# stateless-consensus/phant

Measured on AMD Instinct MI355X. Metric: mpt_proofs_verified_per_sec_depth8, higher is better.
Workload: dtype u64; 1 GPU; config3: 100000 synthetic depth-8 account proofs per GPU against one state root (7 x 532 B full branches + 112 B leaf, 3868 B and 29 Keccak-f per proof, 1% corrupted/exclusion, no cross-proof dedup); every launch sequence in flight verifies its own witness (seeds 2..3: distinct data per slot), 30 back-to-back passes per timed step; parallelism=key-sharded x1, verify_mode=flat, streams=2

## Files before the change

### include/phant_gpu_diag.h

```cpp
#ifndef PHANT_GPU_DIAG_H
#define PHANT_GPU_DIAG_H

#include "phant_gpu.h"

#ifdef __cplusplus
extern "C" {
#endif

PHANT_API int32_t phant_timing(phant_ctx *ctx, int32_t enable);
PHANT_API int32_t phant_last_kernel_ms(phant_ctx *ctx, float *ms);

PHANT_API int32_t phant_verify_stats(phant_ctx *ctx, uint32_t hashed[8]);
PHANT_API int32_t phant_verify_path_stats(phant_ctx *ctx, uint32_t out[2]);
PHANT_API int32_t phant_verify_tier_stats(phant_ctx *ctx, uint32_t out[5]);
PHANT_API int32_t phant_verify_form(phant_ctx *ctx, uint32_t *form);
#define PHANT_VERIFY_KERNEL_STAGES 5
PHANT_API int32_t phant_verify_kernel_ms(phant_ctx *ctx, float ms[PHANT_VERIFY_KERNEL_STAGES]);
PHANT_API int32_t phant_verify_bound_experiment(phant_ctx *ctx, const uint8_t *d_roots, uint32_t n_roots,
                                                const uint32_t *d_root_idx, const uint8_t *d_keys, uint32_t key_len,
                                                const uint8_t *d_nodes, uint64_t nodes_len, const uint64_t *d_node_off,
                                                uint32_t total_nodes, const uint32_t *d_proof_first_node, uint32_t n,
                                                uint8_t *d_status, uint32_t reps, float out_ms[3]);
PHANT_API int32_t phant_keccak_rate(phant_ctx *ctx, uint32_t waves_per_simd, uint32_t perms, double *perms_per_s);

#define PHANT_TRIE_STATS 16
PHANT_API int32_t phant_trie_stats(phant_ctx *ctx, uint32_t out[PHANT_TRIE_STATS]);

PHANT_API int32_t phant_nodeset_tune(phant_ctx *ctx, int32_t form, uint32_t order, uint32_t hash_lds_bytes,
                                     uint32_t resident_wgs);

#define PHANT_NODESET_STATS 14
PHANT_API int32_t phant_nodeset_stats(phant_ctx *ctx, uint32_t out[PHANT_NODESET_STATS]);

#define PHANT_DIAG_SECP_OPS 9
PHANT_API int32_t phant_diag_secp_op(phant_ctx *ctx, uint32_t op, const uint8_t *a, const uint8_t *b, uint32_t n, uint8_t *out);

PHANT_API int32_t phant_diag_scan_u32(phant_ctx *ctx, uint32_t *counters, uint32_t n);
PHANT_API int32_t phant_diag_sort_pairs(phant_ctx *ctx, const uint64_t *keys, const uint32_t *vals, uint32_t n, uint32_t bits,
                                        uint64_t *keys_out, uint32_t *vals_out);
PHANT_API int32_t phant_diag_order_digests(phant_ctx *ctx, const uint8_t *digests, const uint32_t *seg_of, uint32_t n, uint32_t n_seg,
                                           uint32_t prefix_bits, uint32_t *order_out, uint32_t *flag_out);

enum {
    PHANT_DIAG_VERIFY_SERIAL = 1,
    PHANT_DIAG_VERIFY_HASH_LDS_KB,
    PHANT_DIAG_VERIFY_NO_COOP,
    PHANT_DIAG_VERIFY_NO_WAVE,
    PHANT_DIAG_VERIFY_COOP_MAX,
    PHANT_DIAG_STREAM_WGS,
    PHANT_DIAG_STREAM_MB,
    PHANT_DIAG_TRIE_NO_SIDE,
    PHANT_DIAG_TRIE_SIDE_MIN_KEYS,
    PHANT_DIAG_TRIE_AHEAD_MAX_KEYS,
    PHANT_DIAG_TRIE_SIDE_LDS,
    PHANT_DIAG_TRIE_FALLBACK_GRID,
    PHANT_DIAG_TRIE_SLOT_BLOCKS,
    PHANT_DIAG_TRIE_NO_COOP,
    PHANT_DIAG_TRIE_COOP_MAX,
    PHANT_DIAG_TRIE_NO_WAVE,
    PHANT_DIAG_TRIE_JOIN_IN_STREAM,
    PHANT_DIAG_SORT_NO_FALLBACK,
    PHANT_DIAG_SORT_PREFIX_BITS,
    PHANT_DIAG_SORT_REPAIR_BITS,
    PHANT_DIAG_NODESET_WAVE_MAX,
    PHANT_DIAG_TRIE_SMALL_MAX_KEYS,
    PHANT_DIAG_CODE_HASH_FORM,
    PHANT_DIAG_POSTSTATE_RAW_SLOT_KEYS,
    PHANT_DIAG_ADVANCE_ESTIMATE_BYTES,
    PHANT_DIAG_VERIFY_LIST_WGS,
    PHANT_DIAG_RANGES_NO_LEAF_PASS,
    PHANT_DIAG_RANGES_ITEMS_PER_RANGE
};
PHANT_API int32_t phant_diag_set(phant_ctx *ctx, uint32_t knob, int64_t value);

#ifdef __cplusplus
}
#endif
#endif
```

### phant_amd/_lib.py

```python
from __future__ import annotations

import ctypes as C
import os

import torch

_HERE = os.path.dirname(os.path.abspath(__file__))
LIB_PATH = os.path.join(_HERE, "libphant_gpu.so")

OK = 0
E_INVALID_ARG = -1
E_OOM = -2
E_DEVICE = -3
E_NO_DEVICE = -4
E_UNSORTED = -5
E_UNSUPPORTED = -6

PROOF_INVALID_EMPTY = 0
PROOF_PRESENT = 1
PROOF_ABSENT = 2
PROOF_BAD_HASH = 16
PROOF_BAD_RLP = 17
PROOF_BAD_NODE = 18
PROOF_EXTRA_NODES = 19
PROOF_MISSING_NODE = 20
PROOF_BAD_INPUT = 21
PROOF_MISMATCH = 22
PROOF_BAD_VALUE = 23
PROOF_MISSING_SIBLING = 24
RANGE_VALID = 1
RANGE_EMPTY_VALUE = 32
RANGE_VALUE_TOO_LONG = 33
RANGE_BAD_ORDER = 34
RANGE_BELOW_ORIGIN = 35
RANGE_ROOT_MISMATCH = 36
RANGE_NO_LEAF = 0xFFFFFFFF
POST_KEEP, POST_SET, POST_DELETE = 0, 1, 2
PROVE_MAY_REMOVE = 1
ADVANCE_KEEP_OLD = 1
CODE_NONE = 0xFFFFFFFF
SIG_OK, SIG_BAD_RANGE, SIG_HIGH_S, SIG_BAD_RECID, SIG_NOT_ON_CURVE, SIG_INFINITY, SIG_BAD_TX, SIG_BAD_V = range(8)
RECOVER_LOW_S = 1

_vp, _u32, _u64, _i32 = C.c_void_p, C.c_uint32, C.c_uint64, C.c_int32
SYMBOLS = {
    "phant_version": (C.c_char_p, []),
    "phant_device_count": (_i32, []),
    "phant_ctx_create": (_i32, [_vp, C.POINTER(_vp)]),
    "phant_ctx_destroy": (None, [_vp]),
    "phant_last_error": (C.c_char_p, [_vp]),
    "phant_set_stream": (_i32, [_vp, _vp]),
    "phant_stream_sync": (_i32, [_vp]),
    "phant_keccak256": (_i32, [_vp, _vp, _u64, _vp]),
    "phant_keccak256_with_prefix": (_i32, [_vp, _vp, _u64, _vp, _u64, _vp]),
    "phant_keccak256_batch": (_i32, [_vp, _vp, _vp, _u32, _vp]),
    "phant_keccak256_batch_dev": (_i32, [_vp, _vp, _vp, _u32, _vp]),
    "phant_keccak256_fixed_dev": (_i32, [_vp, _vp, _u32, _u64, _u32, _vp]),
    "phant_logs_bloom": (_i32, [_vp, _vp, _vp, _vp, _u32, _u32, _vp]),
    "phant_logs_bloom_dev": (_i32, [_vp, _vp, _vp, _vp, _u32, _u32, _vp]),
    "phant_sender_addresses": (_i32, [_vp, _vp, _u64, _u32, _vp]),
    "phant_sender_addresses_dev": (_i32, [_vp, _vp, _u64, _u32, _vp]),
    "phant_block_receipts": (_i32, [_vp, _vp, _vp]),
    "phant_block_receipts_dev": (_i32, [_vp, _vp, _vp]),
    "phant_header_chain": (_i32, [_vp, _vp, _vp]),
    "phant_header_chain_dev": (_i32, [_vp, _vp, _vp]),
    "phant_headers_decode_rlp": (_i32, [_vp, _vp, _u32, _u32, _vp, _vp]),
    "phant_ecrecover_batch": (_i32, [_vp, _vp, _vp, _vp, _vp, _u32, _u32, _vp, _vp, _vp]),
    "phant_ecrecover_batch_dev": (_i32, [_vp, _vp, _vp, _vp, _vp, _u32, _u32, _vp, _vp, _vp]),
    "phant_tx_senders": (_i32, [_vp, _vp, _vp, _u32, _u64, _vp, _vp]),
    "phant_block_transactions": (_i32, [_vp, _vp, _vp]),
    "phant_block_transactions_dev": (_i32, [_vp, _vp, _vp]),
    "phant_block_transactions_ex": (_i32, [_vp, _vp, _vp]),
    "phant_block_transactions_ex_dev": (_i32, [_vp, _vp, _vp]),
    "phant_block_bodies": (_i32, [_vp, _vp, _vp]),
    "phant_block_bodies_dev": (_i32, [_vp, _vp, _vp]),
    "phant_bodies_decode_rlp": (_i32, [_vp, _vp, _u32, _u32, _vp, _vp]),
    "phant_block_txs_prestate": (_i32, [_vp, _vp, _vp]),
    "phant_block_txs_prestate_dev": (_i32, [_vp, _vp, _vp]),
    "phant_block_settle": (_i32, [_vp, _vp, _vp]),
    "phant_block_settle_dev": (_i32, [_vp, _vp, _vp]),
    "phant_mpt_verify_ranges": (_i32, [_vp, _vp, _vp]),
    "phant_mpt_verify_ranges_dev": (_i32, [_vp, _vp, _vp]),
    "phant_block_access_lists": (_i32, [_vp, _vp, _vp]),
    "phant_block_access_lists_dev": (_i32, [_vp, _vp, _vp]),
    "phant_diag_secp_op": (_i32, [_vp, _u32, _vp, _vp, _u32, _vp]),
    "phant_diag_scan_u32": (_i32, [_vp, _vp, _u32]),
    "phant_diag_sort_pairs": (_i32, [_vp, _vp, _vp, _u32, _u32, _vp, _vp]),
    "phant_diag_order_digests": (_i32, [_vp, _vp, _vp, _u32, _u32, _u32, _vp, _vp]),
    "phant_mpt_verify_batch": (_i32, [_vp, _vp, _u32, _vp, _vp, _u32, _vp, _u64, _vp, _vp, _u32, _vp, _vp, _vp]),
    "phant_mpt_verify_batch_dev": (_i32, [_vp, _vp, _u32, _vp, _vp, _u32, _vp, _u64, _vp, _u32, _vp, _u32, _vp,
                                          _vp, _vp]),
    "phant_mpt_verify_verdict_dev": (_i32, [_vp, _vp, _u32, _vp, _vp, _u32, _vp, _u64, _vp, _u32, _vp, _u32, _vp,
                                            _vp, _vp, _vp]),
    "phant_mpt_verdict_dev": (_i32, [_vp, _vp, _vp, _u32, _u32, _vp]),
    "phant_mpt_verify_nodeset": (_i32, [_vp, _vp, _u32, _vp, _vp, _u32, _vp, _u64, _vp, _u32, _u32, _vp, _vp, _vp]),
    "phant_mpt_verify_nodeset_dev": (_i32, [_vp, _vp, _u32, _vp, _vp, _u32, _vp, _u64, _vp, _u32, _u32, _vp, _vp, _vp]),
    "phant_mpt_verify_nodeset_verdict_dev": (_i32, [_vp, _vp, _u32, _vp, _vp, _u32, _vp, _u64, _vp, _u32, _u32, _vp, _vp, _vp,
                                                    _vp]),
    "phant_mpt_verify_nodeset_submit": (_i32, [_vp, _u32, _vp, _u32, _vp, _vp, _u32, _vp, _u64, _vp, _u32, _u32, _vp, _vp,
                                               _vp]),
    "phant_host_alloc": (_i32, [_vp, C.c_size_t, C.POINTER(_vp)]),
    "phant_host_free": (_i32, [_vp, _vp]),
    "phant_mpt_verify_submit": (_i32, [_vp, _u32, _vp, _u32, _vp, _vp, _u32, _vp, _u64, _vp, _vp, _u32, _vp, _vp, _vp]),
    "phant_wait": (_i32, [_vp, _u32]),
    "phant_witness_parse_json": (_i32, [C.c_char_p, _u64, C.POINTER(_vp), C.c_char_p, _u32]),
    "phant_witness_parse_json_mt": (_i32, [C.c_char_p, _u64, _u32, C.POINTER(_vp), C.c_char_p, _u32]),
    "phant_witness_index_json": (_i32, [C.c_char_p, _u64, _u32, C.POINTER(_vp), C.c_char_p, _u32]),
    "phant_witness_free": (None, [_vp]),
    "phant_witness_get": (_i32, [_vp, _vp]),
    "phant_witness_verify": (_i32, [_vp, _vp, _vp, _vp, C.POINTER(_u32)]),
    "phant_witness_to_json": (_i32, [_vp, _vp, _u64, C.POINTER(_u64)]),
    "phant_exec_witness_parse_json": (_i32, [C.c_char_p, _u64, C.POINTER(_vp), C.c_char_p, _u32]),
    "phant_exec_witness_free": (None, [_vp]),
    "phant_exec_witness_get": (_i32, [_vp, _vp]),
    "phant_exec_witness_prestate": (_i32, [_vp, _vp, _vp, _vp]),
    "phant_exec_witness_poststate": (_i32, [_vp, _vp, _vp, _vp]),
    "phant_exec_witness_advance": (_i32, [_vp, _vp, _vp, _vp, _u32, C.POINTER(_vp)]),
    "phant_mpt_root": (_i32, [_vp, _vp, _vp, _vp, _vp, _u32, _vp]),
    "phant_mpt_root_nodes": (_i32, [_vp, _vp, _vp, _vp, _vp, _u32, _vp, _u32, _vp, _vp, _u32, _vp]),
    "phant_mpt_prove_nodeset": (_i32, [_vp, _vp, _vp, _vp, _vp, _u32, _vp, _u32, _vp, _vp, _vp, _vp, _u32, _vp]),
    "phant_mpt_prove_nodeset_dev": (_i32, [_vp, _vp, _vp, _u64, _vp, _vp, _u64, _u32, _vp, _u32, _vp, _vp, _u64, _vp, _vp, _u32, _vp]),
    "phant_mpt_prove_batch": (_i32, [_vp, _vp, _vp, _vp, _vp, _u32, _vp, _u32, _vp, _vp, _vp, _u32, _vp]),
    "phant_mpt_prove_batch_dev": (_i32, [_vp, _vp, _vp, _u64, _vp, _vp, _u64, _u32, _vp, _u32, _vp, _vp, _u64, _vp, _u32, _vp]),
    "phant_mpt_strip_first_nibble": (_i32, [_vp, _u32, _vp, _u32, C.POINTER(_u32), C.POINTER(_u32)]),
    "phant_index_root_rlp": (_i32, [_vp, _vp, _vp, _u32, _vp]),
    "phant_block_roots": (_i32, [_vp, _vp, _vp, _vp, _u32, _vp, _vp, _vp, _vp, _u32, _u32, _vp]),
    "phant_index_root_be32": (_i32, [_vp, _vp, _vp, _u32, _vp]),
    "phant_state_root": (_i32, [_vp, _vp, _vp, _vp, _vp, _vp, _vp, _vp, _vp, _u32, _vp]),
    "phant_state_witness": (_i32, [_vp, _vp, _vp, _vp, _vp, _vp, _vp, _vp, _vp, _u32, _vp, _vp, _vp, _u32, C.POINTER(_vp), _vp]),
    "phant_state_proofs": (_i32, [_vp, _vp, _vp, _vp, _vp, _vp, _vp, _vp, _vp, _u32, _vp, _vp, _u32, C.POINTER(_vp), _vp]),
    "phant_state_trie_leaves": (_i32, [_vp, _vp, _vp, _vp, _vp, _vp, _vp, _vp, _vp, _u32, _vp, _vp, _u64, _vp]),
    "phant_state_root_dev": (_i32, [_vp, _vp, _vp, _vp, _vp, _vp, _u64, _vp, _vp, _vp, _u32, _u32, _vp]),
    "phant_state_subtrie_nodes": (_i32, [_vp, _vp, _vp, _vp, _vp, _vp, _vp, _vp, _vp, _u32, _vp, _vp, _u32, _vp]),
    "phant_timing": (_i32, [_vp, _i32]),
    "phant_last_kernel_ms": (_i32, [_vp, C.POINTER(C.c_float)]),
    "phant_keccak_rate": (_i32, [_vp, _u32, _u32, C.POINTER(C.c_double)]),
    "phant_nodeset_tune": (_i32, [_vp, _i32, _u32, _u32, _u32]),
    "phant_diag_set": (_i32, [_vp, _u32, C.c_int64]),
    "phant_verify_kernel_ms": (_i32, [_vp, C.POINTER(C.c_float * 5)]),
    "phant_verify_form": (_i32, [_vp, C.POINTER(C.c_uint32)]),
    "phant_verify_bound_experiment": (_i32, [_vp, _vp, _u32, _vp, _vp, _u32, _vp, _u64, _vp, _u32, _vp, _u32, _vp, _u32,
                                            C.POINTER(C.c_float * 3)]),
    "phant_verify_stats": (_i32, [_vp, C.POINTER(C.c_uint32 * 8)]),
    "phant_verify_path_stats": (_i32, [_vp, C.POINTER(C.c_uint32 * 2)]),
    "phant_verify_tier_stats": (_i32, [_vp, C.POINTER(C.c_uint32 * 5)]),
    "phant_trie_stats": (_i32, [_vp, C.POINTER(C.c_uint32 * 16)]),
    "phant_nodeset_stats": (_i32, [_vp, C.POINTER(C.c_uint32 * 14)]),
    "phant_mpt_root_dev": (_i32, [_vp, _vp, _vp, _u64, _vp, _vp, _u64, _u32, _vp]),
    "phant_comm_create": (_i32, [_vp, _u32, _u32, C.POINTER(_vp)]),
    "phant_comm_destroy": (None, [_vp]),
    "phant_comm_size": (_u32, [_vp]),
    "phant_comm_ctx": (_vp, [_vp, _u32]),
    "phant_comm_last_error": (C.c_char_p, [_vp]),
    "phant_comm_owner": (_u32, [_vp, _vp, _u32]),
    "phant_mpt_verify_sharded": (_i32, [_vp, _vp, _u32, _vp, _vp, _u32, _vp, _u64, _vp, _vp, _u32, _vp, _vp, _vp, _vp]),
    "phant_mpt_verify_nodeset_sharded": (_i32, [_vp, _vp, _u32, _vp, _vp, _u32, _vp, _u64, _vp, _u32, _vp, _u32, _vp, _vp, _vp,
                                                _vp]),
    "phant_mpt_root_sharded": (_i32, [_vp, _vp, _vp, _vp, _vp, _u32, _vp]),
    "phant_state_root_sharded": (_i32, [_vp, _vp, _vp, _vp, _vp, _vp, _vp, _vp, _vp, _u32, _vp]),
    "phant_comm_allreduce_verdict": (_i32, [_vp, _vp, _u32]),
}


class PhantOpts(C.Structure):
    _fields_ = [("struct_size", C.c_uint32), ("device", C.c_int32), ("stream", C.c_void_p), ("flags", C.c_uint32)]


class PhantReceiptsIn(C.Structure):
    _fields_ = [("struct_size", C.c_uint32), ("n_receipts", C.c_uint32), ("n_logs", C.c_uint32), ("n_topics", C.c_uint32),
                ("data_bytes", C.c_uint64), ("tx_type", C.c_void_p), ("status", C.c_void_p), ("cum_gas", C.c_void_p),
                ("log_first", C.c_void_p), ("address", C.c_void_p), ("topic_first", C.c_void_p), ("data_off", C.c_void_p),
                ("topics", C.c_void_p), ("data", C.c_void_p), ("lists", C.c_void_p), ("list_off", C.c_void_p),
                ("list_n", C.c_void_p), ("list_bytes", C.c_void_p), ("n_lists", C.c_uint32), ("receipts_at", C.c_uint32)]


class PhantReceiptsOut(C.Structure):
    _fields_ = [("struct_size", C.c_uint32), ("encoded_off_cap", C.c_uint32), ("encoded_cap", C.c_uint64),
                ("receipts_root", C.c_void_p), ("logs_bloom", C.c_void_p), ("blooms", C.c_void_p), ("encoded", C.c_void_p),
                ("encoded_off", C.c_void_p), ("roots_out", C.c_void_p), ("encoded_len", C.c_uint64)]


HEADER_ARRAYS = ("parent_hash", "uncle_hash", "fee_recipient", "state_root", "transactions_root", "receipts_root", "logs_bloom", "difficulty",
                 "number", "gas_limit", "gas_used", "timestamp", "extra_data", "extra_off", "prev_randao", "nonce", "base_fee",
                 "withdrawals_root", "blob_gas_used", "excess_blob_gas", "parent_beacon_root", "requests_hash", "n_fields", "seg_first",
                 "expected_hash")
HEADERS_FROM_BLOCKS = 1


class PhantHeadersIn(C.Structure):
    _fields_ = [("struct_size", C.c_uint32), ("n", C.c_uint32), ("n_segs", C.c_uint32), ("reserved", C.c_uint32)] + \
               [(name, C.c_void_p) for name in HEADER_ARRAYS]


class PhantHeadersOut(C.Structure):
    _fields_ = [("struct_size", C.c_uint32), ("first_bad", C.c_uint32), ("enc_cap", C.c_uint64), ("hashes", C.c_void_p),
                ("flags", C.c_void_p), ("enc", C.c_void_p), ("enc_off", C.c_void_p), ("enc_len", C.c_uint64)]


TXS_HAVE_GAS_LIMIT, TXS_NO_RECOVERY = 1, 2
TX_OUTPUTS = (("tx_hash", "u1", 32), ("sig_hash", "u1", 32), ("sender", "u1", 20), ("sig_status", "u1", 1), ("sig", "u1", 65), ("type", "u1", 1),
              ("chain_id", "u8", 1), ("nonce", "u8", 1), ("gas_limit", "u8", 1), ("gas_price", "u1", 32), ("priority_fee", "u1", 32),
              ("value", "u1", 32), ("to", "u1", 20), ("data_off", "u8", 1), ("data_len", "u4", 1), ("al_off", "u8", 1), ("al_len", "u4", 1),
              ("al_addresses", "u4", 1), ("al_keys", "u4", 1), ("intrinsic_gas", "u8", 1), ("effective_gas_price", "u1", 32),
              ("upfront_cost", "u1", 32), ("flags", "u4", 1))
TX_FLAG_NAMES = ("Undecodable", "BadV", "Signature", "ChainId", "PriorityAboveMax", "FeeBelowBase", "GasAboveBlock", "IntrinsicGas", "NonceMax",
                 "InitcodeSize", "CostOverflow", "IsCreate")
TX_ERROR_BITS = 0x7FF


class PhantTxsIn(C.Structure):
    _fields_ = [("struct_size", C.c_uint32), ("n", C.c_uint32), ("flags", C.c_uint32), ("reserved", C.c_uint32), ("txs", C.c_void_p),
                ("tx_off", C.c_void_p), ("tx_bytes", C.c_uint64), ("chain_id", C.c_uint64), ("base_fee", C.c_void_p),
                ("block_gas_limit", C.c_uint64)]


class PhantTxsOut(C.Structure):
    _fields_ = [("struct_size", C.c_uint32), ("first_bad", C.c_uint32)] + [(name, C.c_void_p) for name, _, _ in TX_OUTPUTS]


TXS_FORK_LONDON, TXS_FORK_CANCUN, TXS_FORK_PRAGUE = 0, 1, 2
AUTH_CHAIN_ID, AUTH_NONCE_MAX = 8, 9
TX_EX_OUTPUTS = (("max_fee_per_blob_gas", "u1", 32), ("blob_off", "u8", 1), ("blobs", "u4", 1), ("auth_first", "u4", 1), ("floor_gas", "u8", 1))
TX_AUTH_OUTPUTS = (("auth_chain_id", "u1", 32), ("auth_address", "u1", 20), ("auth_nonce", "u8", 1), ("auth_hash", "u1", 32), ("auth_sig", "u1", 65),
                   ("authority", "u1", 20), ("auth_status", "u1", 1))
TX_FLAG_NAMES_EX = TX_FLAG_NAMES + ("NoTo", "BlobNone", "BlobVersion", "BlobFeeBelowBase", "AuthNone", "FloorGas")
TX_ERROR_BITS_EX = 0x7FF | 0x7F000


def tx_error_bits(fork=None):
    return TX_ERROR_BITS if fork is None else TX_ERROR_BITS_EX


class PhantTxsExIn(C.Structure):
    _fields_ = [("struct_size", C.c_uint32), ("fork", C.c_uint32), ("base", PhantTxsIn), ("blob_base_fee", C.c_void_p), ("auth_cap", C.c_uint32),
                ("reserved", C.c_uint32)]


class PhantTxsExOut(C.Structure):
    _fields_ = [("struct_size", C.c_uint32), ("n_auth", C.c_uint32), ("blob_gas_used", C.c_uint64), ("base", PhantTxsOut)] + \
               [(name, C.c_void_p) for name, _, _ in TX_EX_OUTPUTS + TX_AUTH_OUTPUTS]


BODY_TX, BODY_TXS_ROOT, BODY_WD_ROOT, BODY_BLOB_GAS = 1, 2, 4, 8
BODY_FLAG_NAMES = ("Transaction", "TransactionsRoot", "WithdrawalsRoot", "BlobGasUsed")
BODIES_INPUTS = ("txs", "tx_off", "block_first", "withdrawals", "wd_off", "wd_first", "base_fee", "gas_limit", "blob_base_fee", "transactions_root",
                 "withdrawals_root", "blob_gas_used")
BODIES_OUTPUTS = (("tx_block", "u4", 1, "n"), ("block_first_bad", "u4", 1, "n_blocks"), ("block_blob_gas_used", "u8", 1, "n_blocks"),
                  ("transactions_root", "u1", 32, "n_blocks"), ("withdrawals_root", "u1", 32, "n_blocks"), ("block_flags", "u4", 1, "n_blocks"))


BODIES_NO_HEADER = 1
BODIES_SPLIT_ARRAYS = ("txs", "tx_off", "block_first", "withdrawals", "wd_off", "wd_first")


class PhantBodiesSplit(C.Structure):
    _fields_ = [(name, C.c_uint32) for name in ("struct_size", "reserved", "tx_cap", "wd_cap")] + [("tx_bytes_cap", C.c_uint64), ("wd_bytes_cap", C.c_uint64)] + \
               [(name, C.c_void_p) for name in BODIES_SPLIT_ARRAYS] + [("n", C.c_uint32), ("n_wd", C.c_uint32), ("tx_bytes", C.c_uint64), ("wd_bytes", C.c_uint64)]


class PhantBodiesIn(C.Structure):
    _fields_ = [(name, C.c_uint32) for name in ("struct_size", "fork", "flags", "n_blocks", "n", "n_wd", "auth_cap", "reserved")] + \
               [("chain_id", C.c_uint64), ("txs", C.c_void_p), ("tx_off", C.c_void_p), ("tx_bytes", C.c_uint64), ("block_first", C.c_void_p),
                ("withdrawals", C.c_void_p), ("wd_off", C.c_void_p), ("wd_bytes", C.c_uint64)] + \
               [(name, C.c_void_p) for name in BODIES_INPUTS[5:]]


class PhantBodiesOut(C.Structure):
    _fields_ = [("struct_size", C.c_uint32), ("first_bad_block", C.c_uint32), ("txs", PhantTxsExOut)] + \
               [(name, C.c_void_p) for name, _, _, _ in BODIES_OUTPUTS]


ROW_NONE = 0xFFFFFFFF
TXSTATE_INPUTS = ("sender", "sig_status", "tx_flags", "nonce", "upfront_cost", "to", "auth_first", "authority", "auth_status", "addresses",
                  "account_status", "nonces", "balances", "code_hashes", "code_index", "code_off", "codes")
TXSTATE_OUTPUTS = (("sender_row", "u4", 1, "n"), ("to_row", "u4", 1, "n"), ("expected_nonce", "u8", 1, "n"), ("spent_before", "u1", 32, "n"),
                   ("state_flags", "u4", 1, "n"), ("sends", "u4", 1, "n_accounts"), ("roles", "u1", 1, "n_accounts"), ("probe_row", "u4", 1, "n_probe"))
TXST_FLAG_NAMES = ("SenderUnknown", "ToUnknown", "NonceLow", "NonceHigh", "BalanceShort", "NotEOA", "CodeMissing", None, "Skipped", "Undetermined",
                   "NeedsInflow", "SpentSaturated")
TXST_ERROR_BITS = 0x7F
TXST_SKIPPED, TXST_UNDETERMINED, TXST_NEEDS_INFLOW, TXST_SPENT_SATURATED = 0x100, 0x200, 0x400, 0x800
ROLE_SENDER, ROLE_RECIPIENT, ROLE_AUTHORITY, ROLE_PROBE = 1, 2, 4, 8


class PhantTxstateIn(C.Structure):
    _fields_ = [(name, C.c_uint32) for name in ("struct_size", "fork", "n", "n_auth", "n_accounts", "n_codes", "n_probe", "reserved")] + \
               [(name, C.c_void_p) for name in TXSTATE_INPUTS] + [("code_bytes", C.c_uint64), ("probe", C.c_void_p)]


class PhantTxstateOut(C.Structure):
    _fields_ = [(name, C.c_uint32) for name in ("struct_size", "first_bad", "n_undetermined", "reserved")] + \
               [(name, C.c_void_p) for name, _, _, _ in TXSTATE_OUTPUTS]


# ... 88 lines not shown
```

### phant_amd/context.py

```python
from __future__ import annotations

import ctypes as C

import numpy as np
import torch

from . import _lib as L


def _np_ptr(a: np.ndarray):
    return a.ctypes.data_as(C.c_void_p)


class Context:

    def __init__(self, device: int | None = None, use_torch_stream: bool = True, verify_nodedup: bool = False,
                 dedup_levels: int | None = None):
        lib = L.lib()
        if not torch.cuda.is_available():
            raise L.PhantError(L.E_NO_DEVICE, "no GPU visible (phant_amd has no CPU fallback)")
        if device is None:
            device = torch.cuda.current_device()
        self.device = int(device)
        stream, flags = None, 1
        if use_torch_stream:
            stream, flags = torch.cuda.current_stream(self.device).cuda_stream or None, 0
        if verify_nodedup:
            dedup_levels = 0
        if dedup_levels is not None:
            flags |= ((int(dedup_levels) + 1) << 8) & 0x1F00
        opts = L.PhantOpts(C.sizeof(L.PhantOpts), self.device, stream, flags)
        h = C.c_void_p()
        rc = lib.phant_ctx_create(C.byref(opts), C.byref(h))
        if rc != L.OK:
            raise L.PhantError(rc, "phant_ctx_create failed (needs a gfx950 device)")
        self._h = h
        self._lib = lib

    @classmethod
    def borrowed(cls, handle, device: int) -> "Context":
        self = cls.__new__(cls)
        self.device = int(device)
        self._lib = L.lib()
        self._h = handle
        self._borrowed = True
        return self

    def check(self, rc: int):
        if rc != L.OK:
            raise L.PhantError(rc, self._lib.phant_last_error(self._h).decode())

    def sync(self):
        self.check(self._lib.phant_stream_sync(self._h))

    def timing(self, enable: bool):
        self.check(self._lib.phant_timing(self._h, 1 if enable else 0))

    def last_kernel_ms(self) -> float:
        ms = C.c_float(0)
        self.check(self._lib.phant_last_kernel_ms(self._h, C.byref(ms)))
        return ms.value

    def keccak_rate(self, waves_per_simd: int = 6, perms: int = 100) -> float:
        out = C.c_double(0.0)
        self.check(self._lib.phant_keccak_rate(self._h, waves_per_simd, perms, C.byref(out)))
        return out.value

    VERIFY_STAGES = ("propose", "hash_deep", "dedup", "hash_list", "walk")
    VERIFY_FORMS = {0: "hash_everything", 1: "two_tiers"}
    DIAG = {name: k + 1 for k, name in enumerate((
        "verify_serial", "verify_hash_lds_kb", "verify_no_coop", "verify_no_wave", "verify_coop_max", "stream_wgs", "stream_mb",
        "trie_no_side", "trie_side_min_keys", "trie_ahead_max_keys", "trie_side_lds", "trie_fallback_grid", "trie_slot_blocks",
        "trie_no_coop", "trie_coop_max", "trie_no_wave", "trie_join_in_stream", "sort_no_fallback", "sort_prefix_bits",
        "sort_repair_bits", "nodeset_wave_max", "trie_small_max_keys", "code_hash_form", "poststate_raw_slot_keys",
        "advance_estimate_bytes", "verify_list_wgs", "ranges_no_leaf_pass", "ranges_items_per_range"))}

    def diag_set(self, knob: str, value: int):
        self.check(self._lib.phant_diag_set(self._h, self.DIAG[knob], int(value)))

    def nodeset_tune(self, form: int = 1, order: int = 0, hash_lds: int = 40 * 1024, resident_wgs: int = 0):
        self.check(self._lib.phant_nodeset_tune(self._h, form, order, hash_lds, resident_wgs))

    def verify_kernel_ms(self) -> dict[str, float]:
        out = (C.c_float * 5)()
        self.check(self._lib.phant_verify_kernel_ms(self._h, C.byref(out)))
        return dict(zip(self.VERIFY_STAGES, [float(x) for x in out]))

    def verify_bound_experiment(self, batch, reps: int = 20) -> dict[str, float]:
        import torch
        st = torch.empty(batch.n, dtype=torch.uint8, device=batch.nodes.device)
        out = (C.c_float * 3)()
        self.check(self._lib.phant_verify_bound_experiment(
            self._h, batch.roots.data_ptr(), batch.n_roots, None if batch.root_idx is None else batch.root_idx.data_ptr(),
            batch.keys.data_ptr(), batch.key_len, batch.nodes.data_ptr(), batch.nodes.numel(), batch.node_off.data_ptr(),
            batch.node_off.numel() - 1, batch.proof_first_node.data_ptr(), batch.n, st.data_ptr(), reps, C.byref(out)))
        return {"hash_only_ms": float(out[0]), "stream_only_ms": float(out[1]), "together_ms": float(out[2])}

    def verify_form(self) -> str:
        out = C.c_uint32(0)
        self.check(self._lib.phant_verify_form(self._h, C.byref(out)))
        return self.VERIFY_FORMS.get(int(out.value), "?")

    def verify_stats(self) -> list[int]:
        out = (C.c_uint32 * 8)()
        self.check(self._lib.phant_verify_stats(self._h, C.byref(out)))
        return list(out)

    def verify_tier_stats(self) -> dict[str, int]:
        out = (C.c_uint32 * 5)()
        self.check(self._lib.phant_verify_tier_stats(self._h, C.byref(out)))
        return dict(zip(("dedup_levels", "list_nodes", "list_keccak_f", "deep_nodes", "deep_keccak_f"), [int(x) for x in out]))

    TRIE_PASSES = {0: "none", 1: "small", 2: "general"}

    def trie_stats(self) -> dict:
        out = (C.c_uint32 * 16)()
        self.check(self._lib.phant_trie_stats(self._h, C.byref(out)))
        v = [int(x) for x in out]
        return {"pass": self.TRIE_PASSES.get(v[0], "?"), "leaves_ahead": bool(v[1]), "deep_from": v[2] - (1 << 32) if v[2] >> 31 else v[2],
                "bins": v[3], "max_bin": v[4], "wave": v[5], "half_wave": v[6], "blocks1": v[7], "blocks2": v[8], "blocks4": v[9],
                "misfits": v[10], "leaf_big": bool(v[11]), "n_rep": v[12], "n": v[13], "side_bins": v[14], "scratch_bytes": v[15]}

    def nodeset_stats(self) -> list[int]:
        out = (C.c_uint32 * 14)()
        self.check(self._lib.phant_nodeset_stats(self._h, C.byref(out)))
        return [int(x) for x in out]

    def verify_path_stats(self) -> tuple[int, int]:
        out = (C.c_uint32 * 2)()
        self.check(self._lib.phant_verify_path_stats(self._h, C.byref(out)))
        return int(out[0]), int(out[1])

    def close(self):
        if getattr(self, "_h", None):
            if not getattr(self, "_borrowed", False):
                self._lib.phant_ctx_destroy(self._h)
            self._h = None

    def __del__(self):
        try:
            self.close()
        except Exception:
            pass

    @property
    def handle(self):
        return self._h


_default: dict[int, Context] = {}


def default_context(device: int | None = None) -> Context:
    if device is None:
        device = torch.cuda.current_device() if torch.cuda.is_available() else 0
    ctx = _default.get(device)
    if ctx is None:
        ctx = Context(device)
        _default[device] = ctx
    return ctx
```

### phant_amd/csrc/capi.hip

```cpp
#include <hip/hip_runtime.h>

#include <algorithm>
#include <cstdio>
#include <cstdlib>
#include <cstring>
#include <memory>
#include <new>
#include <random>
#include <string>
#include <vector>

#include "../../include/phant_gpu.h"
#include "../../include/phant_gpu_diag.h"
#include "arena.h"
#include "staging.h"
#include "launch.h"
#include "receipts.h"
#include "headers.h"
#include "transactions.h"
#include "settle.h"
#include "txstate.h"
#include "access_lists.h"
#include "trie_build.h"
#include "witness.h"
// ... 168 lines not shown
    DeviceGuard g(dev);
    if (!own) {
        c->stream = (hipStream_t)stream;
    } else {
        if (hipStreamCreateWithFlags(&c->stream, hipStreamNonBlocking) != hipSuccess) {
            c->stream = nullptr;
            return PHANT_E_DEVICE;
        }
        c->own_stream = true;
    }
    if (hipEventCreate(&c->ev0) != hipSuccess || hipEventCreate(&c->ev1) != hipSuccess) return PHANT_E_DEVICE;
    c->tune.last_shallow = &c->last_shallow;
    c->tune.last_form = &c->last_form;
    holder.c = nullptr;
    *out = c;
    return PHANT_OK;
}

void phant_ctx_destroy(phant_ctx* c) {
    if (!c) return;
    DeviceGuard g(c->device);
    (void)hipStreamSynchronize(c->stream);
    c->ws.release();
    c->dv.release();
    c->ns.dv.release();
    if (c->secp_gtable) (void)hipFree(c->secp_gtable);
    if (c->ev0) (void)hipEventDestroy(c->ev0);
    if (c->ev1) (void)hipEventDestroy(c->ev1);
    for (hipEvent_t e : c->kev)
        if (e) (void)hipEventDestroy(e);
    for (auto& sl : c->slots) {
        if (sl.stream) {
            (void)hipStreamSynchronize(sl.stream);
            (void)hipStreamDestroy(sl.stream);
        }
        sl.io.release();
        sl.dv.release();
        sl.ns.dv.release();
    }
    if (c->side.stream) (void)hipStreamSynchronize(c->side.stream);
    if (c->side.stream2) (void)hipStreamSynchronize(c->side.stream2);
    if (c->side.fork) (void)hipEventDestroy(c->side.fork);
    if (c->side.join) (void)hipEventDestroy(c->side.join);
    if (c->side.join2) (void)hipEventDestroy(c->side.join2);
    if (c->code_side.stream) (void)hipStreamSynchronize(c->code_side.stream);
    if (c->code_side.fork) (void)hipEventDestroy(c->code_side.fork);
    if (c->code_side.join) (void)hipEventDestroy(c->code_side.join);
    if (c->code_side.stream) (void)hipStreamDestroy(c->code_side.stream);
    if (c->side.stream) (void)hipStreamDestroy(c->side.stream);
    if (c->side.stream2) (void)hipStreamDestroy(c->side.stream2);
    if (c->own_stream && c->stream) (void)hipStreamDestroy(c->stream);
    delete c;
}

const char* phant_last_error(const phant_ctx* c) { return c ? c->err.c_str() : "null ctx"; }

int32_t phant_set_stream(phant_ctx* c, void* stream) {
    if (!c) return PHANT_E_INVALID_ARG;
    DeviceGuard g(c->device);
    HIP_TRY(c, hipStreamSynchronize(c->stream));
    if (c->own_stream) {
        (void)hipStreamDestroy(c->stream);
        c->own_stream = false;
    }
    c->stream = (hipStream_t)stream;
    return PHANT_OK;
}

int32_t phant_stream_sync(phant_ctx* c) {
    if (!c) return PHANT_E_INVALID_ARG;
    DeviceGuard g(c->device);
    HIP_TRY(c, hipStreamSynchronize(c->stream));
    return PHANT_OK;
}

int32_t phant_timing(phant_ctx* c, int32_t enable) {
    if (!c) return PHANT_E_INVALID_ARG;
    c->timing = enable != 0;
    c->ev_pending = false;
    return PHANT_OK;
}

int32_t phant_verify_stats(phant_ctx* c, uint32_t hashed[8]) {
    if (!c || !hashed) return PHANT_E_INVALID_ARG;
    for (int i = 0; i < 8; ++i) hashed[i] = 0;
    if (c->last_was_nodeset) {
        if (!c->ns.dv.base) return PHANT_OK;
        DeviceGuard g(c->device);
        HIP_TRY(c, hipStreamSynchronize(c->stream));
        uint32_t hdr[phant::VERIFY_HEADER_WORDS];
        HIP_TRY(c, hipMemcpy(hdr, c->ns.dv.base, sizeof(hdr), hipMemcpyDeviceToHost));
        phant::verify_nodeset_stats_from_header(hdr, c->ns.epoch, hashed, nullptr);
        return PHANT_OK;
    }
    if (!c->dv.base) return PHANT_OK;
    DeviceGuard g(c->device);
    HIP_TRY(c, hipStreamSynchronize(c->stream));
    if (c->side.stream) HIP_TRY(c, hipStreamSynchronize(c->side.stream));
    uint32_t hdr[phant::VERIFY_HEADER_WORDS];
    HIP_TRY(c, hipMemcpy(hdr, c->dv.base, sizeof(hdr), hipMemcpyDeviceToHost));
    phant::verify_stats_from_header(hdr, hashed);
    return PHANT_OK;
}

int32_t phant_nodeset_stats(phant_ctx* c, uint32_t out[PHANT_NODESET_STATS]) {
    if (!c || !out) return PHANT_E_INVALID_ARG;
    for (int i = 0; i < PHANT_NODESET_STATS; ++i) out[i] = 0;
    if (!c->ns.dv.base || c->ns.dirty || c->ns.epoch == 0u || c->ns_last[0] == 0u) return PHANT_OK;
    DeviceGuard g(c->device);
    HIP_TRY(c, hipStreamSynchronize(c->stream));
    uint32_t hdr[phant::VERIFY_HEADER_WORDS];
    HIP_TRY(c, hipMemcpy(hdr, c->ns.dv.base, sizeof(hdr), hipMemcpyDeviceToHost));
    uint32_t hashed[8], overflow = 0;
    phant::verify_nodeset_stats_from_header(hdr, c->ns.epoch, hashed, &overflow);
    phant::verify_nodeset_lists_from_header(hdr, c->ns.epoch, out + 1);
    out[0] = c->ns_last[0];
    out[10] = overflow;
    out[11] = c->ns_last[1];
    out[12] = c->ns_last[2];
    out[13] = c->ns.epoch;
    return PHANT_OK;
}

int32_t phant_verify_tier_stats(phant_ctx* c, uint32_t out[5]) {
    if (!c || !out) return PHANT_E_INVALID_ARG;
    for (int i = 0; i < 5; ++i) out[i] = 0;
    if (!c->dv.base) return PHANT_OK;
    DeviceGuard g(c->device);
    HIP_TRY(c, hipStreamSynchronize(c->stream));
    if (c->side.stream) HIP_TRY(c, hipStreamSynchronize(c->side.stream));
    uint32_t hdr[phant::VERIFY_HEADER_WORDS];
    HIP_TRY(c, hipMemcpy(hdr, c->dv.base, sizeof(hdr), hipMemcpyDeviceToHost));
    out[0] = c->last_shallow;
    phant::verify_tier_stats_from_header(hdr, out + 1);
    return PHANT_OK;
}

int32_t phant_verify_form(phant_ctx* c, uint32_t* form) {
    if (!c || !form) return PHANT_E_INVALID_ARG;
    *form = c->last_form;
    return PHANT_OK;
}

int32_t phant_verify_path_stats(phant_ctx* c, uint32_t out[2]) {
    if (!c || !out) return PHANT_E_INVALID_ARG;
    out[0] = out[1] = 0;
    if (!c->dv.base) return PHANT_OK;
    DeviceGuard g(c->device);
    HIP_TRY(c, hipStreamSynchronize(c->stream));
    if (c->side.stream) HIP_TRY(c, hipStreamSynchronize(c->side.stream));
    uint32_t hdr[phant::VERIFY_HEADER_WORDS];
    HIP_TRY(c, hipMemcpy(hdr, c->dv.base, sizeof(hdr), hipMemcpyDeviceToHost));
    phant::verify_paths_from_header(hdr, out);
    return PHANT_OK;
}

int32_t phant_trie_stats(phant_ctx* c, uint32_t out[PHANT_TRIE_STATS]) {
    if (!c || !out) return PHANT_E_INVALID_ARG;
    const phant::TrieStats& s = c->ws.trie_stats;
    for (int i = 0; i < PHANT_TRIE_STATS; ++i) out[i] = 0;
    out[0] = s.pass;
    out[1] = s.ahead;
    out[2] = (uint32_t)s.deep_from;
    out[3] = s.bins;
    out[4] = s.max_bin;
    for (int k = 0; k < 5; ++k) out[5 + k] = s.by_class[k];
    out[11] = s.leaf_big;
    out[12] = s.n_rep;
    out[13] = s.n;
    out[14] = s.side_bins;
    DeviceGuard g(c->device);
    HIP_TRY(c, hipStreamSynchronize(c->stream));
    if (c->ws.side) HIP_TRY(c, hipStreamSynchronize(c->ws.side));
    constexpr size_t MISFIT_BYTES = 512 * sizeof(uint32_t);
    if (s.has_misfit && c->ws.t1.base && s.misfit_off + MISFIT_BYTES <= c->ws.t1.cap) {
        std::vector<uint32_t> mis(512);
        HIP_TRY(c, hipMemcpy(mis.data(), c->ws.t1.base + s.misfit_off, MISFIT_BYTES, hipMemcpyDeviceToHost));
        uint64_t tot = 0;
        for (const uint32_t m : mis) tot += m;
        out[10] = (uint32_t)std::min<uint64_t>(tot, 0xffffffffull);
    }
    if (s.has_cursor && c->ws.t1.base && s.cursor_off + sizeof(unsigned long long) <= c->ws.t1.cap) {
        unsigned long long used = 0;
        HIP_TRY(c, hipMemcpy(&used, c->ws.t1.base + s.cursor_off, sizeof used, hipMemcpyDeviceToHost));
        out[15] = (uint32_t)std::min<unsigned long long>(used, 0xffffffffull);
    }
    return PHANT_OK;
}

int32_t phant_verify_kernel_ms(phant_ctx* c, float ms[PHANT_VERIFY_KERNEL_STAGES]) {
    if (!c || !ms) return PHANT_E_INVALID_ARG;
    if (!c->tune.kernel_ev) return fail(c, PHANT_E_UNSUPPORTED, "verify_kernel_ms: the tiers are not serialised on this ctx (phant_diag_set: the verify-serial knob)");
    if (!c->kev_valid) return fail(c, PHANT_E_INVALID_ARG, "verify_kernel_ms: the last verify launch on this ctx was not a two-tier one");
    DeviceGuard g(c->device);
    HIP_TRY(c, hipStreamSynchronize(c->stream));
    static_assert(PHANT_VERIFY_KERNEL_STAGES == phant::VERIFY_KERNEL_STAGES, "one stage list");
    for (int i = 0; i < PHANT_VERIFY_KERNEL_STAGES; ++i) {
        ms[i] = 0.f;
        if (hipEventElapsedTime(&ms[i], c->kev[i], c->kev[i + 1]) != hipSuccess) {
            (void)hipGetLastError();
            return fail(c, PHANT_E_INVALID_ARG, "verify_kernel_ms: no two-tier launch on this ctx yet");
        }
    }
    return PHANT_OK;
}

int32_t phant_last_kernel_ms(phant_ctx* c, float* ms) {
    if (!c || !ms) return PHANT_E_INVALID_ARG;
    if (!c->ev_pending) return fail(c, PHANT_E_INVALID_ARG, "no timed call pending");
    DeviceGuard g(c->device);
    HIP_TRY(c, hipEventSynchronize(c->ev1));
    HIP_TRY(c, hipEventElapsedTime(ms, c->ev0, c->ev1));
    return PHANT_OK;
}

int32_t phant_diag_set(phant_ctx* c, uint32_t knob, int64_t value) {
    if (!c) return PHANT_E_INVALID_ARG;
    DeviceGuard g(c->device);
    phant::TrieTune& t = c->ws.tune;
    switch (knob) {
        case PHANT_DIAG_VERIFY_SERIAL:
            if (value && !c->tune.kernel_ev) {
                for (hipEvent_t& e : c->kev)
                    if (!e) HIP_TRY(c, hipEventCreate(&e));
                c->tune.kernel_ev = c->kev;
            }
            c->tune.serial = value != 0;
            c->kev_valid = false;
            return PHANT_OK;
        case PHANT_DIAG_VERIFY_HASH_LDS_KB:
            c->tune.hash_lds = (uint32_t)(value < 0 ? 0 : value > 47 ? 47 : value) * 1024u;
            return PHANT_OK;
        case PHANT_DIAG_VERIFY_NO_COOP: c->tune.no_coop = value != 0; return PHANT_OK;
        case PHANT_DIAG_VERIFY_NO_WAVE: c->tune.no_wave = value != 0; return PHANT_OK;
        case PHANT_DIAG_VERIFY_COOP_MAX: c->tune.coop_max = (uint32_t)(value < 0 ? 0 : value > (1 << 20) ? (1 << 20) : value); return PHANT_OK;
        case PHANT_DIAG_STREAM_WGS: c->tune.diag_stream_wgs = (uint32_t)(value < 0 ? 0 : value > 65536 ? 65536 : value); return PHANT_OK;
        case PHANT_DIAG_STREAM_MB: c->tune.diag_stream_mb = (uint32_t)(value < 0 ? 0 : value > 65536 ? 65536 : value); return PHANT_OK;
        case PHANT_DIAG_TRIE_NO_SIDE: t.no_side = value != 0; return PHANT_OK;
        case PHANT_DIAG_TRIE_SIDE_MIN_KEYS: t.side_min_keys = value; return PHANT_OK;
        case PHANT_DIAG_TRIE_AHEAD_MAX_KEYS: t.ahead_max_keys = value; return PHANT_OK;
        case PHANT_DIAG_TRIE_SIDE_LDS: t.side_lds = value; return PHANT_OK;
        case PHANT_DIAG_TRIE_FALLBACK_GRID: t.fallback_grid = value; return PHANT_OK;
        case PHANT_DIAG_TRIE_SLOT_BLOCKS: t.slot_blocks = (int32_t)value; return PHANT_OK;
        case PHANT_DIAG_TRIE_NO_COOP: t.no_coop = value != 0; return PHANT_OK;
        case PHANT_DIAG_TRIE_COOP_MAX: t.coop_max = value; return PHANT_OK;
        case PHANT_DIAG_TRIE_NO_WAVE: t.no_wave = value != 0; return PHANT_OK;
        case PHANT_DIAG_TRIE_JOIN_IN_STREAM: t.join_in_stream = value != 0; return PHANT_OK;
        case PHANT_DIAG_SORT_NO_FALLBACK: t.sort_no_fallback = value != 0; return PHANT_OK;
        case PHANT_DIAG_SORT_PREFIX_BITS: t.sort_prefix_bits = value; return PHANT_OK;
        case PHANT_DIAG_SORT_REPAIR_BITS: t.sort_repair_bits = value; return PHANT_OK;
        case PHANT_DIAG_NODESET_WAVE_MAX: c->ns_tune.wave_max = (uint32_t)(value < 0 ? 0 : value > (1 << 20) ? (1 << 20) : value); return PHANT_OK;
        case PHANT_DIAG_TRIE_SMALL_MAX_KEYS: t.small_max_keys = value; return PHANT_OK;
        case PHANT_DIAG_CODE_HASH_FORM: c->code_form = value == 1 ? 1u : 0u; return PHANT_OK;
        case PHANT_DIAG_POSTSTATE_RAW_SLOT_KEYS: c->post_raw_slot_keys = value != 0; return PHANT_OK;
        case PHANT_DIAG_ADVANCE_ESTIMATE_BYTES: c->advance_estimate = value > 0 ? (uint64_t)value : 0u; return PHANT_OK;
        case PHANT_DIAG_VERIFY_LIST_WGS: c->tune.list_wgs_cap = (uint32_t)(value < 0 ? 0 : value > (1 << 20) ? (1 << 20) : value); return PHANT_OK;
        case PHANT_DIAG_RANGES_NO_LEAF_PASS: c->ranges_no_leaf_pass = value != 0; return PHANT_OK;
        case PHANT_DIAG_RANGES_ITEMS_PER_RANGE: c->ranges_items_per_range = value < 0 ? -1 : value > 1922 ? 1922 : value; return PHANT_OK;
        default: return fail(c, PHANT_E_INVALID_ARG, "diag_set: no such knob");
    }
}

int32_t phant_nodeset_tune(phant_ctx* c, int32_t ladder, uint32_t order, uint32_t hash_lds_bytes, uint32_t resident_wgs) {
    if (!c || ladder < 0 || ladder > 2 || order > 1u || hash_lds_bytes > 56u * 1024u) return PHANT_E_INVALID_ARG;
    c->ns_tune.form = (uint32_t)ladder;
    c->ns_tune.order = order;
    c->ns_tune.hash_lds = hash_lds_bytes;
    c->ns_tune.resident_wgs = resident_wgs;
    return PHANT_OK;
}

int32_t phant_keccak_rate(phant_ctx* c, uint32_t waves_per_simd, uint32_t perms, double* perms_per_s) {
    if (!c || !perms_per_s || waves_per_simd == 0 || waves_per_simd > 8 || perms == 0) return PHANT_E_INVALID_ARG;
    DeviceGuard g(c->device);
    int cus = 0;
    HIP_TRY(c, hipDeviceGetAttribute(&cus, hipDeviceAttributeMultiprocessorCount, c->device));
    const uint32_t blocks = (uint32_t)cus * waves_per_simd;
    uint32_t* d_out = nullptr;
    const int32_t rc = lay_out(c, c->stream, c->ws.io, [&](auto& io) { d_out = io.template take<uint32_t>((size_t)blocks * 256); });
    if (rc) return rc;
    hipEvent_t e0 = nullptr, e1 = nullptr;
    HIP_TRY(c, hipEventCreate(&e0));
    hipError_t e = hipEventCreate(&e1);
    if (e == hipSuccess) e = phant::launch_keccak_rate(d_out, blocks, perms, c->stream);
    if (e == hipSuccess) e = hipEventRecord(e0, c->stream);
    if (e == hipSuccess) e = phant::launch_keccak_rate(d_out, blocks, perms, c->stream);
    if (e == hipSuccess) e = hipEventRecord(e1, c->stream);
    if (e == hipSuccess) e = hipEventSynchronize(e1);
    float ms = 0.f;
    if (e == hipSuccess) e = hipEventElapsedTime(&ms, e0, e1);
    (void)hipEventDestroy(e0);
    if (e1) (void)hipEventDestroy(e1);
    if (e != hipSuccess) return fail(c, PHANT_E_DEVICE, "keccak_rate", e);
    *perms_per_s = ms > 0.f ? (double)blocks * 256.0 * perms / (ms * 1e-3) : 0.0;
    return PHANT_OK;
}


int32_t phant_keccak256_batch_dev(phant_ctx* c, const uint8_t* d_blob, const uint64_t* d_off,
                                  uint32_t n, uint8_t* d_out) {
    if (!c) return PHANT_E_INVALID_ARG;
    if (n == 0) return PHANT_OK;
    if (!d_off || !d_out || !aligned16(d_out)) return fail(c, PHANT_E_INVALID_ARG, "keccak256_batch_dev: null or unaligned pointer");
    DeviceGuard g(c->device);
    TimedRegion t(c);
    HIP_TRY(c, phant::launch_keccak256_var(d_blob, d_off, n, d_out, c->stream));
    return PHANT_OK;
}

int32_t phant_keccak256_fixed_dev(phant_ctx* c, const uint8_t* d_blob, uint32_t msg_len,
                                  uint64_t stride, uint32_t n, uint8_t* d_out) {
    if (!c) return PHANT_E_INVALID_ARG;
    if (n == 0) return PHANT_OK;
    if (!d_out || !aligned16(d_out) || (!d_blob && msg_len) || (stride < msg_len && n > 1))
        return fail(c, PHANT_E_INVALID_ARG, "keccak256_fixed_dev: bad argument");
    DeviceGuard g(c->device);
    TimedRegion t(c);
    HIP_TRY(c, phant::launch_keccak256_fixed(d_blob, msg_len, stride, n, d_out, c->stream));
    return PHANT_OK;
}

int32_t phant_keccak256_batch(phant_ctx* c, const uint8_t* blob, const uint64_t* off, uint32_t n,
                              uint8_t* out) {
    if (!c) return PHANT_E_INVALID_ARG;
    if (n == 0) return PHANT_OK;
    if (!off || !out) return fail(c, PHANT_E_INVALID_ARG, "keccak256_batch: null pointer");
    for (uint32_t i = 0; i < n; ++i)
        if (off[i + 1] < off[i]) return fail(c, PHANT_E_INVALID_ARG, "keccak256_batch: offsets not monotone");
    const uint64_t lo = off[0], hi = off[n];
    const size_t blob_len = (size_t)(hi - lo);
    if (blob_len && !blob) return fail(c, PHANT_E_INVALID_ARG, "keccak256_batch: null blob");
    DeviceGuard g(c->device);
    uint8_t *d_blob = nullptr, *d_out = nullptr;
    uint64_t* d_off = nullptr;
    const int32_t rc = lay_out(c, c->stream, c->ws.io, [&](auto& io) {
        d_blob = io.template take<uint8_t>(blob_len + 16);
        d_off = io.template take<uint64_t>((size_t)n + 1);
        d_out = io.template take<uint8_t>((size_t)n * 32);
    });
    if (rc) return rc;
    std::vector<uint64_t> rel((size_t)n + 1);
    for (uint32_t i = 0; i <= n; ++i) rel[i] = off[i] - lo;
    if (blob_len) HIP_TRY(c, hipMemcpyAsync(d_blob, blob + lo, blob_len, hipMemcpyHostToDevice, c->stream));
    HIP_TRY(c, hipMemcpyAsync(d_off, rel.data(), rel.size() * 8, hipMemcpyHostToDevice, c->stream));
    HIP_TRY(c, phant::launch_keccak256_var(d_blob, d_off, n, d_out, c->stream));
    HIP_TRY(c, hipMemcpyAsync(out, d_out, (size_t)n * 32, hipMemcpyDeviceToHost, c->stream));
    HIP_TRY(c, hipStreamSynchronize(c->stream));
    return PHANT_OK;
}

int32_t phant_keccak256(phant_ctx* c, const uint8_t* data, uint64_t len, uint8_t out[32]) {
    const uint64_t off[2] = {0, len};
    return phant_impl::phant_keccak256_batch(c, data, off, 1, out);
}

int32_t phant_keccak256_with_prefix(phant_ctx* c, const uint8_t* prefix, uint64_t prefix_len,
                                    const uint8_t* data, uint64_t len, uint8_t out[32]) {
    if (!c) return PHANT_E_INVALID_ARG;
    if ((prefix_len && !prefix) || (len && !data)) return fail(c, PHANT_E_INVALID_ARG, "keccak256_with_prefix: null pointer");
    uint8_t* cat = (uint8_t*)std::malloc((size_t)(prefix_len + len) + 1);
    if (!cat) return fail(c, PHANT_E_OOM, "keccak256_with_prefix: host staging");
    if (prefix_len) std::memcpy(cat, prefix, (size_t)prefix_len);
    if (len) std::memcpy(cat + prefix_len, data, (size_t)len);
    const uint64_t off[2] = {0, prefix_len + len};
    const int32_t rc = phant_impl::phant_keccak256_batch(c, cat, off, 1, out);
    std::free(cat);
    return rc;
}


int32_t phant_logs_bloom_dev(phant_ctx* c, const uint8_t* d_items, const uint64_t* d_item_off,
                             const uint32_t* d_item_receipt, uint32_t n_items, uint32_t n_receipts, uint8_t* d_blooms) {
    if (!c) return PHANT_E_INVALID_ARG;
    if (n_receipts == 0) return PHANT_OK;
    if (!d_blooms || ((uintptr_t)d_blooms & 3u) || (n_items && (!d_item_off || !d_item_receipt)))
        return fail(c, PHANT_E_INVALID_ARG, "logs_bloom_dev: null or unaligned pointer");
    DeviceGuard g(c->device);
    TimedRegion t(c);
    HIP_TRY(c, phant::launch_logs_bloom(d_items, d_item_off, d_item_receipt, n_items, n_receipts, d_blooms, c->stream));
    return PHANT_OK;
}

int32_t phant_logs_bloom(phant_ctx* c, const uint8_t* items, const uint64_t* item_off, const uint32_t* item_receipt,
                         uint32_t n_items, uint32_t n_receipts, uint8_t* blooms) {
    if (!c) return PHANT_E_INVALID_ARG;
    if (n_receipts == 0) return PHANT_OK;
    if (!blooms || (n_items && (!item_off || !item_receipt))) return fail(c, PHANT_E_INVALID_ARG, "logs_bloom: null pointer");
    for (uint32_t i = 0; i < n_items; ++i)
        if (item_off[i + 1] < item_off[i]) return fail(c, PHANT_E_INVALID_ARG, "logs_bloom: offsets not monotone");
    const uint64_t lo = n_items ? item_off[0] : 0, hi = n_items ? item_off[n_items] : 0;
    const size_t blob_len = (size_t)(hi - lo);
    if (blob_len && !items) return fail(c, PHANT_E_INVALID_ARG, "logs_bloom: null items");
    DeviceGuard g(c->device);
    uint8_t *d_items = nullptr, *d_blooms = nullptr;
    uint64_t* d_off = nullptr;
    uint32_t* d_rcpt = nullptr;
    const int32_t rc = lay_out(c, c->stream, c->ws.io, [&](auto& io) {
        d_items = io.template take<uint8_t>(blob_len + 16);
        d_off = io.template take<uint64_t>((size_t)n_items + 1);
        d_rcpt = io.template take<uint32_t>((size_t)n_items + 1);
        d_blooms = io.template take<uint8_t>((size_t)n_receipts * 256);
    });
    if (rc) return rc;
    std::vector<uint64_t> rel((size_t)n_items + 1, 0);
    for (uint32_t i = 0; i <= n_items && n_items; ++i) rel[i] = item_off[i] - lo;
    if (blob_len) HIP_TRY(c, hipMemcpyAsync(d_items, items + lo, blob_len, hipMemcpyHostToDevice, c->stream));
    HIP_TRY(c, hipMemcpyAsync(d_off, rel.data(), rel.size() * 8, hipMemcpyHostToDevice, c->stream));
    if (n_items) HIP_TRY(c, hipMemcpyAsync(d_rcpt, item_receipt, (size_t)n_items * 4, hipMemcpyHostToDevice, c->stream));
    HIP_TRY(c, phant::launch_logs_bloom(d_items, d_off, d_rcpt, n_items, n_receipts, d_blooms, c->stream));
// ... 2200 lines not shown
```

### phant_amd/csrc/capi_guard_capi.inc

```
extern "C" {

const char * phant_version(void) {
    try { return phant_impl::phant_version(); } catch (...) { return nullptr; }
}

int32_t phant_device_count(void) {
    try { return phant_impl::phant_device_count(); }
    catch (const std::bad_alloc&) { return phant_impl::guard_failed(nullptr, PHANT_E_OOM); }
    catch (...) { return phant_impl::guard_failed(nullptr, PHANT_E_DEVICE); }
}

int32_t phant_ctx_create(const phant_opts *opts, phant_ctx **out) {
    try { return phant_impl::phant_ctx_create(opts, out); }
    catch (const std::bad_alloc&) { return phant_impl::guard_failed(nullptr, PHANT_E_OOM); }
    catch (...) { return phant_impl::guard_failed(nullptr, PHANT_E_DEVICE); }
}

void phant_ctx_destroy(phant_ctx *ctx) {
    try { phant_impl::phant_ctx_destroy(ctx); } catch (...) {}
}

const char * phant_last_error(const phant_ctx *ctx) {
    try { return phant_impl::phant_last_error(ctx); } catch (...) { return nullptr; }
}
// ... 330 lines not shown
    catch (...) { return phant_impl::guard_failed(ctx, PHANT_E_DEVICE); }
}

int32_t phant_exec_witness_advance(phant_ctx *ctx, const phant_exec_witness *w, const uint8_t *parent_state_root, phant_poststate *io, uint32_t flags, phant_exec_witness **next) {
    try { return phant_impl::phant_exec_witness_advance(ctx, w, parent_state_root, io, flags, next); }
    catch (const std::bad_alloc&) { return phant_impl::guard_failed(ctx, PHANT_E_OOM); }
    catch (...) { return phant_impl::guard_failed(ctx, PHANT_E_DEVICE); }
}

int32_t phant_mpt_root(phant_ctx *ctx, const uint8_t *keys, const uint32_t *key_off, const uint8_t *vals, const uint64_t *val_off, uint32_t n, uint8_t out[32]) {
    try { return phant_impl::phant_mpt_root(ctx, keys, key_off, vals, val_off, n, out); }
    catch (const std::bad_alloc&) { return phant_impl::guard_failed(ctx, PHANT_E_OOM); }
    catch (...) { return phant_impl::guard_failed(ctx, PHANT_E_DEVICE); }
}

int32_t phant_mpt_root_dev(phant_ctx *ctx, const uint8_t *d_keys, const uint32_t *d_key_off, uint64_t key_bytes, const uint8_t *d_vals, const uint64_t *d_val_off, uint64_t val_bytes, uint32_t n, uint8_t *d_root) {
    try { return phant_impl::phant_mpt_root_dev(ctx, d_keys, d_key_off, key_bytes, d_vals, d_val_off, val_bytes, n, d_root); }
    catch (const std::bad_alloc&) { return phant_impl::guard_failed(ctx, PHANT_E_OOM); }
    catch (...) { return phant_impl::guard_failed(ctx, PHANT_E_DEVICE); }
}

int32_t phant_mpt_prove_nodeset(phant_ctx *ctx, const uint8_t *keys, const uint32_t *key_off, const uint8_t *vals, const uint64_t *val_off, uint32_t n, const uint32_t *seg_first , uint32_t n_tries, const uint8_t *qkeys, const uint32_t *qkey_off , const uint32_t *q_trie , const uint8_t *q_flags , uint32_t n_queries, phant_prove_out *out) {
    try { return phant_impl::phant_mpt_prove_nodeset(ctx, keys, key_off, vals, val_off, n, seg_first, n_tries, qkeys, qkey_off, q_trie, q_flags, n_queries, out); }
    catch (const std::bad_alloc&) { return phant_impl::guard_failed(ctx, PHANT_E_OOM); }
    catch (...) { return phant_impl::guard_failed(ctx, PHANT_E_DEVICE); }
}

int32_t phant_mpt_prove_nodeset_dev(phant_ctx *ctx, const uint8_t *d_keys, const uint32_t *d_key_off, uint64_t key_bytes, const uint8_t *d_vals, const uint64_t *d_val_off, uint64_t val_bytes, uint32_t n, const uint32_t *d_seg_first , uint32_t n_tries, const uint8_t *d_qkeys, const uint32_t *d_qkey_off, uint64_t qkey_bytes, const uint32_t *d_q_trie , const uint8_t *d_q_flags , uint32_t n_queries, phant_prove_out *out) {
    try { return phant_impl::phant_mpt_prove_nodeset_dev(ctx, d_keys, d_key_off, key_bytes, d_vals, d_val_off, val_bytes, n, d_seg_first, n_tries, d_qkeys, d_qkey_off, qkey_bytes, d_q_trie, d_q_flags, n_queries, out); }
    catch (const std::bad_alloc&) { return phant_impl::guard_failed(ctx, PHANT_E_OOM); }
    catch (...) { return phant_impl::guard_failed(ctx, PHANT_E_DEVICE); }
}

int32_t phant_mpt_prove_batch(phant_ctx *ctx, const uint8_t *keys, const uint32_t *key_off, const uint8_t *vals, const uint64_t *val_off, uint32_t n, const uint32_t *seg_first , uint32_t n_tries, const uint8_t *qkeys, const uint32_t *qkey_off , const uint32_t *q_trie , uint32_t n_queries, phant_prove_batch_out *out) {
    try { return phant_impl::phant_mpt_prove_batch(ctx, keys, key_off, vals, val_off, n, seg_first, n_tries, qkeys, qkey_off, q_trie, n_queries, out); }
    catch (const std::bad_alloc&) { return phant_impl::guard_failed(ctx, PHANT_E_OOM); }
    catch (...) { return phant_impl::guard_failed(ctx, PHANT_E_DEVICE); }
}

int32_t phant_mpt_prove_batch_dev(phant_ctx *ctx, const uint8_t *d_keys, const uint32_t *d_key_off, uint64_t key_bytes, const uint8_t *d_vals, const uint64_t *d_val_off, uint64_t val_bytes, uint32_t n, const uint32_t *d_seg_first , uint32_t n_tries, const uint8_t *d_qkeys, const uint32_t *d_qkey_off, uint64_t qkey_bytes, const uint32_t *d_q_trie , uint32_t n_queries, phant_prove_batch_out *out) {
    try { return phant_impl::phant_mpt_prove_batch_dev(ctx, d_keys, d_key_off, key_bytes, d_vals, d_val_off, val_bytes, n, d_seg_first, n_tries, d_qkeys, d_qkey_off, qkey_bytes, d_q_trie, n_queries, out); }
    catch (const std::bad_alloc&) { return phant_impl::guard_failed(ctx, PHANT_E_OOM); }
    catch (...) { return phant_impl::guard_failed(ctx, PHANT_E_DEVICE); }
}

int32_t phant_index_root_rlp(phant_ctx *ctx, const uint8_t *items, const uint64_t *item_off, uint32_t n, uint8_t out[32]) {
    try { return phant_impl::phant_index_root_rlp(ctx, items, item_off, n, out); }
    catch (const std::bad_alloc&) { return phant_impl::guard_failed(ctx, PHANT_E_OOM); }
    catch (...) { return phant_impl::guard_failed(ctx, PHANT_E_DEVICE); }
}

int32_t phant_index_root_be32(phant_ctx *ctx, const uint8_t *items, const uint64_t *item_off, uint32_t n, uint8_t out[32]) {
    try { return phant_impl::phant_index_root_be32(ctx, items, item_off, n, out); }
    catch (const std::bad_alloc&) { return phant_impl::guard_failed(ctx, PHANT_E_OOM); }
    catch (...) { return phant_impl::guard_failed(ctx, PHANT_E_DEVICE); }
}

int32_t phant_block_roots(phant_ctx *ctx, const uint8_t *const *items, const uint64_t *const *item_off, const uint32_t *n, uint32_t n_lists, uint8_t *roots_out, const uint8_t *bloom_items, const uint64_t *bloom_item_off, const uint32_t *bloom_item_receipt, uint32_t n_bloom_items, uint32_t n_receipts, uint8_t *blooms) {
    try { return phant_impl::phant_block_roots(ctx, items, item_off, n, n_lists, roots_out, bloom_items, bloom_item_off, bloom_item_receipt, n_bloom_items, n_receipts, blooms); }
    catch (const std::bad_alloc&) { return phant_impl::guard_failed(ctx, PHANT_E_OOM); }
    catch (...) { return phant_impl::guard_failed(ctx, PHANT_E_DEVICE); }
}

int32_t phant_mpt_verify_ranges(phant_ctx *ctx, const phant_ranges_in *in, phant_ranges_out *out) {
    try { return phant_impl::phant_mpt_verify_ranges(ctx, in, out); }
    catch (const std::bad_alloc&) { return phant_impl::guard_failed(ctx, PHANT_E_OOM); }
    catch (...) { return phant_impl::guard_failed(ctx, PHANT_E_DEVICE); }
}

int32_t phant_mpt_verify_ranges_dev(phant_ctx *ctx, const phant_ranges_in *in, phant_ranges_out *out) {
    try { return phant_impl::phant_mpt_verify_ranges_dev(ctx, in, out); }
    catch (const std::bad_alloc&) { return phant_impl::guard_failed(ctx, PHANT_E_OOM); }
    catch (...) { return phant_impl::guard_failed(ctx, PHANT_E_DEVICE); }
}

int32_t phant_mpt_root_nodes(phant_ctx *ctx, const uint8_t *keys, const uint32_t *key_off, const uint8_t *vals, const uint64_t *val_off, uint32_t n, const uint32_t *seg_first , uint32_t n_tries, uint8_t *roots , uint8_t *node_rlp , uint32_t node_cap, uint32_t *node_len) {
    try { return phant_impl::phant_mpt_root_nodes(ctx, keys, key_off, vals, val_off, n, seg_first, n_tries, roots, node_rlp, node_cap, node_len); }
    catch (const std::bad_alloc&) { return phant_impl::guard_failed(ctx, PHANT_E_OOM); }
    catch (...) { return phant_impl::guard_failed(ctx, PHANT_E_DEVICE); }
}

int32_t phant_mpt_strip_first_nibble(const uint8_t *node, uint32_t len, uint8_t *out, uint32_t cap, uint32_t *out_len, uint32_t *is_ref) {
    try { return phant_impl::phant_mpt_strip_first_nibble(node, len, out, cap, out_len, is_ref); }
    catch (const std::bad_alloc&) { return phant_impl::guard_failed(nullptr, PHANT_E_OOM); }
    catch (...) { return phant_impl::guard_failed(nullptr, PHANT_E_DEVICE); }
}

int32_t phant_state_root(phant_ctx *ctx, const uint8_t *addrs, const uint64_t *nonces, const uint8_t *balances, const uint8_t *code, const uint64_t *code_off, const uint8_t *slot_keys, const uint8_t *slot_vals, const uint32_t *slot_first, uint32_t n, uint8_t out[32]) {
    try { return phant_impl::phant_state_root(ctx, addrs, nonces, balances, code, code_off, slot_keys, slot_vals, slot_first, n, out); }
    catch (const std::bad_alloc&) { return phant_impl::guard_failed(ctx, PHANT_E_OOM); }
    catch (...) { return phant_impl::guard_failed(ctx, PHANT_E_DEVICE); }
}

int32_t phant_state_root_dev(phant_ctx *ctx, const uint8_t *d_addrs, const uint64_t *d_nonces, const uint8_t *d_balances, const uint8_t *d_code, const uint64_t *d_code_off, uint64_t code_bytes, const uint8_t *d_slot_keys, const uint8_t *d_slot_vals, const uint32_t *d_slot_first, uint32_t n_slots, uint32_t n, uint8_t *d_root) {
    try { return phant_impl::phant_state_root_dev(ctx, d_addrs, d_nonces, d_balances, d_code, d_code_off, code_bytes, d_slot_keys, d_slot_vals, d_slot_first, n_slots, n, d_root); }
    catch (const std::bad_alloc&) { return phant_impl::guard_failed(ctx, PHANT_E_OOM); }
    catch (...) { return phant_impl::guard_failed(ctx, PHANT_E_DEVICE); }
}

int32_t phant_state_witness(phant_ctx *ctx, const uint8_t *addrs, const uint64_t *nonces, const uint8_t *balances, const uint8_t *code, const uint64_t *code_off, const uint8_t *slot_keys, const uint8_t *slot_vals, const uint32_t *slot_first, uint32_t n, const uint8_t *wkeys, const uint32_t *wkey_off , const uint8_t *wkey_flags , uint32_t n_wkeys, phant_exec_witness **out, uint8_t state_root_out[32]) {
    try { return phant_impl::phant_state_witness(ctx, addrs, nonces, balances, code, code_off, slot_keys, slot_vals, slot_first, n, wkeys, wkey_off, wkey_flags, n_wkeys, out, state_root_out); }
    catch (const std::bad_alloc&) { return phant_impl::guard_failed(ctx, PHANT_E_OOM); }
    catch (...) { return phant_impl::guard_failed(ctx, PHANT_E_DEVICE); }
}

int32_t phant_state_proofs(phant_ctx *ctx, const uint8_t *addrs, const uint64_t *nonces, const uint8_t *balances, const uint8_t *code, const uint64_t *code_off, const uint8_t *slot_keys, const uint8_t *slot_vals, const uint32_t *slot_first, uint32_t n, const uint8_t *wkeys, const uint32_t *wkey_off , uint32_t n_wkeys, phant_witness **out, uint8_t state_root_out[32]) {
    try { return phant_impl::phant_state_proofs(ctx, addrs, nonces, balances, code, code_off, slot_keys, slot_vals, slot_first, n, wkeys, wkey_off, n_wkeys, out, state_root_out); }
    catch (const std::bad_alloc&) { return phant_impl::guard_failed(ctx, PHANT_E_OOM); }
    catch (...) { return phant_impl::guard_failed(ctx, PHANT_E_DEVICE); }
}

int32_t phant_state_subtrie_nodes(phant_ctx *ctx, const uint8_t *addrs, const uint64_t *nonces, const uint8_t *balances, const uint8_t *code, const uint64_t *code_off, const uint8_t *slot_keys, const uint8_t *slot_vals, const uint32_t *slot_first, uint32_t n, uint8_t *roots, uint8_t *root_enc, uint32_t root_enc_cap, uint32_t *root_enc_len) {
    try { return phant_impl::phant_state_subtrie_nodes(ctx, addrs, nonces, balances, code, code_off, slot_keys, slot_vals, slot_first, n, roots, root_enc, root_enc_cap, root_enc_len); }
    catch (const std::bad_alloc&) { return phant_impl::guard_failed(ctx, PHANT_E_OOM); }
    catch (...) { return phant_impl::guard_failed(ctx, PHANT_E_DEVICE); }
}

int32_t phant_state_trie_leaves(phant_ctx *ctx, const uint8_t *addrs, const uint64_t *nonces, const uint8_t *balances, const uint8_t *code, const uint64_t *code_off, const uint8_t *slot_keys, const uint8_t *slot_vals, const uint32_t *slot_first, uint32_t n, uint8_t *keys, uint8_t *vals, uint64_t vals_cap, uint64_t *val_off) {
    try { return phant_impl::phant_state_trie_leaves(ctx, addrs, nonces, balances, code, code_off, slot_keys, slot_vals, slot_first, n, keys, vals, vals_cap, val_off); }
    catch (const std::bad_alloc&) { return phant_impl::guard_failed(ctx, PHANT_E_OOM); }
    catch (...) { return phant_impl::guard_failed(ctx, PHANT_E_DEVICE); }
}

int32_t phant_timing(phant_ctx *ctx, int32_t enable) {
    try { return phant_impl::phant_timing(ctx, enable); }
    catch (const std::bad_alloc&) { return phant_impl::guard_failed(ctx, PHANT_E_OOM); }
    catch (...) { return phant_impl::guard_failed(ctx, PHANT_E_DEVICE); }
}

int32_t phant_last_kernel_ms(phant_ctx *ctx, float *ms) {
    try { return phant_impl::phant_last_kernel_ms(ctx, ms); }
    catch (const std::bad_alloc&) { return phant_impl::guard_failed(ctx, PHANT_E_OOM); }
    catch (...) { return phant_impl::guard_failed(ctx, PHANT_E_DEVICE); }
}

int32_t phant_verify_stats(phant_ctx *ctx, uint32_t hashed[8]) {
    try { return phant_impl::phant_verify_stats(ctx, hashed); }
    catch (const std::bad_alloc&) { return phant_impl::guard_failed(ctx, PHANT_E_OOM); }
    catch (...) { return phant_impl::guard_failed(ctx, PHANT_E_DEVICE); }
}

int32_t phant_verify_path_stats(phant_ctx *ctx, uint32_t out[2]) {
    try { return phant_impl::phant_verify_path_stats(ctx, out); }
    catch (const std::bad_alloc&) { return phant_impl::guard_failed(ctx, PHANT_E_OOM); }
    catch (...) { return phant_impl::guard_failed(ctx, PHANT_E_DEVICE); }
}

int32_t phant_verify_tier_stats(phant_ctx *ctx, uint32_t out[5]) {
    try { return phant_impl::phant_verify_tier_stats(ctx, out); }
    catch (const std::bad_alloc&) { return phant_impl::guard_failed(ctx, PHANT_E_OOM); }
    catch (...) { return phant_impl::guard_failed(ctx, PHANT_E_DEVICE); }
}

int32_t phant_verify_form(phant_ctx *ctx, uint32_t *form) {
    try { return phant_impl::phant_verify_form(ctx, form); }
    catch (const std::bad_alloc&) { return phant_impl::guard_failed(ctx, PHANT_E_OOM); }
    catch (...) { return phant_impl::guard_failed(ctx, PHANT_E_DEVICE); }
}

int32_t phant_verify_kernel_ms(phant_ctx *ctx, float ms[PHANT_VERIFY_KERNEL_STAGES]) {
    try { return phant_impl::phant_verify_kernel_ms(ctx, ms); }
    catch (const std::bad_alloc&) { return phant_impl::guard_failed(ctx, PHANT_E_OOM); }
    catch (...) { return phant_impl::guard_failed(ctx, PHANT_E_DEVICE); }
}

int32_t phant_verify_bound_experiment(phant_ctx *ctx, const uint8_t *d_roots, uint32_t n_roots, const uint32_t *d_root_idx, const uint8_t *d_keys, uint32_t key_len, const uint8_t *d_nodes, uint64_t nodes_len, const uint64_t *d_node_off, uint32_t total_nodes, const uint32_t *d_proof_first_node, uint32_t n, uint8_t *d_status, uint32_t reps, float out_ms[3]) {
    try { return phant_impl::phant_verify_bound_experiment(ctx, d_roots, n_roots, d_root_idx, d_keys, key_len, d_nodes, nodes_len, d_node_off, total_nodes, d_proof_first_node, n, d_status, reps, out_ms); }
    catch (const std::bad_alloc&) { return phant_impl::guard_failed(ctx, PHANT_E_OOM); }
    catch (...) { return phant_impl::guard_failed(ctx, PHANT_E_DEVICE); }
}

int32_t phant_keccak_rate(phant_ctx *ctx, uint32_t waves_per_simd, uint32_t perms, double *perms_per_s) {
    try { return phant_impl::phant_keccak_rate(ctx, waves_per_simd, perms, perms_per_s); }
    catch (const std::bad_alloc&) { return phant_impl::guard_failed(ctx, PHANT_E_OOM); }
    catch (...) { return phant_impl::guard_failed(ctx, PHANT_E_DEVICE); }
}

int32_t phant_trie_stats(phant_ctx *ctx, uint32_t out[PHANT_TRIE_STATS]) {
    try { return phant_impl::phant_trie_stats(ctx, out); }
    catch (const std::bad_alloc&) { return phant_impl::guard_failed(ctx, PHANT_E_OOM); }
    catch (...) { return phant_impl::guard_failed(ctx, PHANT_E_DEVICE); }
}

int32_t phant_nodeset_tune(phant_ctx *ctx, int32_t form, uint32_t order, uint32_t hash_lds_bytes, uint32_t resident_wgs) {
    try { return phant_impl::phant_nodeset_tune(ctx, form, order, hash_lds_bytes, resident_wgs); }
    catch (const std::bad_alloc&) { return phant_impl::guard_failed(ctx, PHANT_E_OOM); }
    catch (...) { return phant_impl::guard_failed(ctx, PHANT_E_DEVICE); }
}

int32_t phant_nodeset_stats(phant_ctx *ctx, uint32_t out[PHANT_NODESET_STATS]) {
    try { return phant_impl::phant_nodeset_stats(ctx, out); }
    catch (const std::bad_alloc&) { return phant_impl::guard_failed(ctx, PHANT_E_OOM); }
    catch (...) { return phant_impl::guard_failed(ctx, PHANT_E_DEVICE); }
}

int32_t phant_diag_secp_op(phant_ctx *ctx, uint32_t op, const uint8_t *a, const uint8_t *b, uint32_t n, uint8_t *out) {
    try { return phant_impl::phant_diag_secp_op(ctx, op, a, b, n, out); }
    catch (const std::bad_alloc&) { return phant_impl::guard_failed(ctx, PHANT_E_OOM); }
    catch (...) { return phant_impl::guard_failed(ctx, PHANT_E_DEVICE); }
}

int32_t phant_diag_scan_u32(phant_ctx *ctx, uint32_t *counters, uint32_t n) {
    try { return phant_impl::phant_diag_scan_u32(ctx, counters, n); }
    catch (const std::bad_alloc&) { return phant_impl::guard_failed(ctx, PHANT_E_OOM); }
    catch (...) { return phant_impl::guard_failed(ctx, PHANT_E_DEVICE); }
}

int32_t phant_diag_sort_pairs(phant_ctx *ctx, const uint64_t *keys, const uint32_t *vals, uint32_t n, uint32_t bits, uint64_t *keys_out, uint32_t *vals_out) {
    try { return phant_impl::phant_diag_sort_pairs(ctx, keys, vals, n, bits, keys_out, vals_out); }
    catch (const std::bad_alloc&) { return phant_impl::guard_failed(ctx, PHANT_E_OOM); }
    catch (...) { return phant_impl::guard_failed(ctx, PHANT_E_DEVICE); }
}

int32_t phant_diag_order_digests(phant_ctx *ctx, const uint8_t *digests, const uint32_t *seg_of, uint32_t n, uint32_t n_seg, uint32_t prefix_bits, uint32_t *order_out, uint32_t *flag_out) {
    try { return phant_impl::phant_diag_order_digests(ctx, digests, seg_of, n, n_seg, prefix_bits, order_out, flag_out); }
    catch (const std::bad_alloc&) { return phant_impl::guard_failed(ctx, PHANT_E_OOM); }
    catch (...) { return phant_impl::guard_failed(ctx, PHANT_E_DEVICE); }
}

int32_t phant_diag_set(phant_ctx *ctx, uint32_t knob, int64_t value) {
    try { return phant_impl::phant_diag_set(ctx, knob, value); }
    catch (const std::bad_alloc&) { return phant_impl::guard_failed(ctx, PHANT_E_OOM); }
    catch (...) { return phant_impl::guard_failed(ctx, PHANT_E_DEVICE); }
}

}
```

### phant_amd/csrc/launch.h

```cpp
#pragma once
#include <hip/hip_runtime.h>
#include <stdint.h>

namespace phant {

hipError_t launch_keccak256_var(const uint8_t* d_blob, const uint64_t* d_off, uint32_t n,
                                uint8_t* d_out, hipStream_t st);
hipError_t launch_keccak256_fixed(const uint8_t* d_blob, uint32_t msg_len, uint64_t stride,
                                  uint32_t n, uint8_t* d_out, hipStream_t st);

hipError_t launch_keccak_rate(uint32_t* d_out, uint32_t blocks, uint32_t perms, hipStream_t st);

hipError_t launch_logs_bloom(const uint8_t* d_items, const uint64_t* d_item_off, const uint32_t* d_item_receipt,
                             uint32_t n_items, uint32_t n_receipts, uint8_t* d_blooms, hipStream_t st);
hipError_t launch_sender_addresses(const uint8_t* d_pubkeys, uint64_t stride, uint32_t n, uint8_t* d_out,
                                   hipStream_t st);

constexpr size_t SECP_GTABLE_BYTES = 256 * 64;
hipError_t launch_secp_gtable(uint32_t* d_gtable, hipStream_t st);
hipError_t launch_ecrecover(const uint8_t* d_hashes, const uint8_t* d_r, const uint8_t* d_s, const uint8_t* d_recid,
                            const uint8_t* d_pre_status, uint32_t n, uint32_t flags, const uint32_t* d_gtable,
                            uint8_t* d_pubkeys, uint8_t* d_addresses, uint8_t* d_status, hipStream_t st);
hipError_t launch_secp_op(uint32_t op, const uint8_t* d_a, const uint8_t* d_b, uint32_t n, uint8_t* d_out, hipStream_t st);

hipError_t launch_hex_decode(const uint8_t* d_json, const uint64_t* d_node_src, const uint64_t* d_node_off,
                             uint32_t total_nodes, uint8_t* d_nodes, uint32_t* d_err, hipStream_t st);
hipError_t launch_gather_values(const uint8_t* d_nodes, const uint64_t* d_value_off, const uint32_t* d_value_len,
                                uint32_t n, uint32_t cap, uint8_t* d_out, hipStream_t st);

struct VerifyArgs {
    const uint8_t* roots;
    uint32_t n_roots;
    const uint32_t* root_idx;
    const uint8_t* keys;
    uint32_t key_len;
    const uint8_t* nodes;
    uint64_t nodes_len;
    const uint64_t* node_off;
    const uint32_t* proof_first_node;
    uint32_t n;
    uint8_t* status;
    uint64_t* value_off;
    uint32_t* value_len;
    uint32_t* fail_count = nullptr;
    uint32_t total_nodes = 0;
};
struct FlatSide {
    hipStream_t stream;
    hipEvent_t fork, join;
    hipStream_t stream2 = nullptr;
    hipEvent_t join2 = nullptr;
};
size_t verify_workspace_bytes(uint32_t total_nodes);
struct VerifyTune {
    uint32_t hash_lds = 40u * 1024u;
    bool serial = false;
    uint32_t* last_shallow = nullptr;
    hipEvent_t* kernel_ev = nullptr;
    uint32_t coop_max = 2048;
    bool no_coop = false;
    bool no_wave = false;
    uint32_t* last_form = nullptr;
    uint32_t list_wgs_cap = 0;
    uint32_t diag = 0;
    uint32_t* diag_sink = nullptr;
    uint32_t diag_stream_wgs = 0;
    uint32_t diag_stream_mb = 0;
};
constexpr int VERIFY_KERNEL_STAGES = 5;
hipError_t launch_mpt_verify(const VerifyArgs& a, uint32_t total_nodes, uint8_t* ws, int32_t dedup_levels,
                             hipStream_t st, const FlatSide* side, const VerifyTune& tune);
constexpr uint32_t VERIFY_HEADER_WORDS = 2048;
void verify_stats_from_header(const uint32_t* hdr, uint32_t hashed[8]);
void verify_tier_stats_from_header(const uint32_t* hdr, uint32_t out[4]);
void verify_paths_from_header(const uint32_t* hdr, uint32_t out[2]);
struct NodesetTune {
    uint32_t form = 1;
    uint32_t order = 0;
    uint32_t hash_lds = 40u * 1024u;
    uint32_t wave_max = 3500;
    uint32_t resident_wgs = 0;
    uint32_t* last = nullptr;
};
uint32_t verify_nodeset_capacity(uint32_t total_nodes);
size_t verify_nodeset_workspace_bytes(uint32_t cap_nodes);
hipError_t launch_mpt_verify_nodeset(const VerifyArgs& a, uint32_t total_nodes, uint32_t cap_nodes, uint8_t* ws, uint32_t epoch,
                                     const uint32_t salt[2], hipStream_t st, const NodesetTune& tune);
void verify_nodeset_stats_from_header(const uint32_t* hdr, uint32_t epoch, uint32_t hashed[8], uint32_t* overflow);
void verify_nodeset_lists_from_header(const uint32_t* hdr, uint32_t epoch, uint32_t lists[9]);
struct PrestateArgs {
    const uint8_t* nodes;
    uint32_t na, ns, nc;
    uint8_t* acc_status;
    const uint64_t* acc_voff;
    const uint32_t* acc_vlen;
    uint64_t* nonces;
    uint8_t* balances;
    uint8_t* storage_roots;
    uint8_t* code_hashes;
    uint32_t* code_index;
    uint8_t* slot_status;
    const uint64_t* slot_voff;
    const uint32_t* slot_vlen;
    const uint32_t* slot_account;
    uint8_t* slot_vals;
    uint32_t* counters;
    const uint8_t* codes;
    const uint64_t* code_off;
    uint32_t* code_dig;
    uint32_t* code_slot;
    uint32_t* table;
    uint32_t* table_used;
    uint32_t mask;
    uint32_t salt0, salt1;
};
enum : uint32_t { PRE_CNT_FAILED = 0, PRE_CNT_MISSING_CODE = 1, PRE_CNT_UNUSED_CODES = 2 };
hipError_t launch_prestate_accounts(const PrestateArgs& a, hipStream_t st);
hipError_t launch_prestate_slots(const PrestateArgs& a, hipStream_t st);
hipError_t launch_code_hash(const PrestateArgs& a, uint32_t form, hipStream_t st);
hipError_t launch_code_match(const PrestateArgs& a, hipStream_t st);
uint32_t code_table_slots(uint32_t n_codes);
hipError_t launch_nodeset_hash(const VerifyArgs& a, uint32_t total_nodes, uint32_t cap_nodes, uint8_t* ws, uint32_t epoch,
                               const uint32_t salt[2], hipStream_t st, const NodesetTune& tune);
hipError_t launch_nodeset_walk(const VerifyArgs& a, uint32_t cap_nodes, uint8_t* ws, uint32_t epoch, const uint32_t salt[2],
                               hipStream_t st);
struct PoststateNodeDesc {
    uint64_t off;
    uint32_t len, trie, item, where;
};
struct PoststateArgs {
    const uint8_t* nodes;
    uint64_t nodes_len;
    uint32_t na, ns;
    const uint8_t* keys;
    const uint8_t* parent_root;
    uint8_t* acc_status;
    uint8_t* slot_status;
    const uint64_t* acc_voff;
    const uint32_t* acc_vlen;
    const uint64_t* slot_voff;
    const uint32_t* slot_vlen;
    const uint64_t* pre_nonces;
    const uint8_t* pre_balances;
    const uint8_t* pre_sroots;
    const uint8_t* pre_code_hashes;
    const uint32_t* slot_account;
    const uint32_t* slot_first;
    const uint8_t* op;
    const uint64_t* post_nonces;
    const uint8_t* post_balances;
    const uint8_t* post_code_hashes;
    const uint8_t* slot_write;
    const uint8_t* post_slot_vals;
    uint8_t* post_sroots;
    uint8_t* state_root;
    uint32_t* acc_flag;
    uint8_t* act;
    uint32_t* seg_of;
    const uint32_t* order;
    uint8_t* key_bad;
    uint32_t* cnt;
    uint32_t* scan_scratch;
    void* items_raw;
    uint32_t cap_items;
    uint32_t* counters;
    uint8_t* sink_blob;
    PoststateNodeDesc* sink_desc;
    unsigned long long* sink_bytes;
    uint32_t* sink_cnt;
    const uint32_t* sink_undecided;
    uint64_t sink_cap_bytes;
    uint32_t sink_cap_desc;
    uint32_t* trie_bad;
    const uint8_t* leaf_vals;
};
constexpr size_t POSTSTATE_ITEM_BYTES = 96;
enum : uint32_t { POST_SINK_NODES = 0, POST_SINK_OVERFLOW = 1 };
enum : uint32_t { POST_CNT_ITEMS = 3, POST_CNT_INTERNAL = 4, POST_CNT_EMIT_FAILED = 5 };
hipError_t launch_poststate_actions(const PoststateArgs& p, hipStream_t st);
hipError_t launch_poststate_build(const PoststateArgs& p, uint32_t cap_nodes, uint8_t* ws, uint32_t epoch, const uint32_t salt[2],
                                  hipStream_t st);
struct RangeArgs {
    uint32_t n_ranges, n_leaves, n_nodes;
    const uint8_t* roots;
    const uint8_t* origins;
    const uint32_t* leaf_first;
    const uint8_t* has_proof;
    const uint8_t* keys;
    const uint8_t* vals;
    const uint64_t* val_off;
    uint64_t vals_len;
    const uint8_t* nodes;
    const uint64_t* node_off;
    uint64_t nodes_len;
    uint32_t* ctl;
    uint32_t* counters;
    uint32_t* bad_leaf;
    uint32_t* walk_err;
    uint32_t* more;
    uint32_t* trie_bad;
    uint8_t* built_root;
    uint32_t* cnt;
    uint32_t* scan_scratch;
    void* items_raw;
    uint32_t cap_items;
    uint32_t leaf_pass;
    uint8_t* status;
    uint8_t* has_more;
    uint8_t* computed_root;
    uint32_t* out_bad_leaf;
};
enum : uint32_t { RANGE_CTL_CHECK = 0, RANGE_CTL_FAILED = 1, RANGE_CTL_FIRST = 2, RANGE_CTL_ITEMS = 3, RANGE_CTL_WORDS = 4 };
hipError_t launch_range_check(const RangeArgs& a, hipStream_t st);
hipError_t launch_range_verify(const RangeArgs& a, uint32_t cap_nodes, uint8_t* ws, uint32_t epoch, const uint32_t salt[2], hipStream_t st);
hipError_t launch_mpt_verdict(const uint8_t* d_status, const uint32_t* d_root_idx, uint32_t n,
                              uint32_t n_roots, uint32_t* d_fail_count, hipStream_t st);

size_t order_workspace_bytes(uint32_t n);
hipError_t launch_order_digests(const uint8_t* d_digests, const uint32_t* d_seg_of, uint32_t n, uint32_t n_seg, uint8_t* ws,
                                uint32_t** d_order_out, uint32_t** d_flag_out, uint32_t prefix_bits, hipStream_t st);

size_t sort_hist_entries(uint32_t n);
hipError_t launch_sort_pairs(uint64_t* keys, uint32_t* vals, uint64_t* keys_alt, uint32_t* vals_alt, uint32_t n, uint32_t bits, uint32_t* hist,
                             uint32_t* digit_totals, uint64_t** keys_out, uint32_t** vals_out, hipStream_t st);
inline uint32_t sort_key_bits(uint32_t n_accounts) {
    uint32_t bits = 1;
    while (bits < 32u && (n_accounts >> bits)) ++bits;
    return bits;
// ... 7 lines not shown
```

### phant_amd/csrc/mpt_verify_v3.hip

```cpp
#include <phant_platform.h>

#include "launch.h"
#include "mpt_verify_one.hip.h"
#include "coop_sponge.hip.h"
#include "verify_hash.hip.h"

namespace phant {
namespace v3 {
using namespace vh;

constexpr uint32_t HDR_PFN_BROKEN = 9;
constexpr uint32_t HDR_SLOW = 10;
constexpr uint32_t HDR_OPENED = 11;
constexpr uint32_t HDR_PARITY = 15;
constexpr uint32_t HDR_STAT = 1024;
constexpr uint32_t HDR_STAT_STRIPES = 16;
constexpr uint32_t HDR_STAT_WORDS = HDR_STAT_STRIPES * N_CLASS;
constexpr uint32_t HDR_STAT_END = HDR_STAT + 2u * HDR_STAT_WORDS;
constexpr uint32_t HDR_CUR = 256;
constexpr uint32_t HDR_WORDS = 768;
constexpr size_t HEADER_BYTES = 8192;
static_assert(HDR_STAT_END <= VERIFY_HEADER_WORDS && 4u * VERIFY_HEADER_WORDS <= HEADER_BYTES,
              "capi.hip copies VERIFY_HEADER_WORDS words back for the statistics");

PHANT_DEV uint32_t cursor_word(uint32_t cls, uint32_t stripe) { return HDR_CUR + 32u * stripe + cls; }



PHANT_DEV uint64_t key_prefix64(const uint8_t* __restrict__ key, uint32_t key_len) {
    uint64_t kb = 0;
    const uint32_t take = key_len < 8u ? key_len : 8u;
    for (uint32_t t = 0; t < take; ++t) kb |= (uint64_t)key[t] << (56u - 8u * t);
    return kb;
}
PHANT_DEV uint64_t key_prefix64_wide(const uint8_t* __restrict__ key, uint32_t key_len) {
    if (key_len < 8u) return key_prefix64(key, key_len);
    struct __attribute__((packed, aligned(1))) U64u { unsigned long long v; };
    return __builtin_bswap64(reinterpret_cast<const U64u*>(key)->v);
}
PHANT_DEV bool same_prefix(uint64_t x, uint64_t y, uint32_t d) { return d == 0u || ((x ^ y) >> (64u - 4u * d)) == 0ull; }
PHANT_DEV uint64_t group_hash(uint64_t kb, uint32_t root, uint32_t d) {
    const uint64_t pre = d ? (kb >> (64u - 4u * d)) : 0ull;
    uint64_t h = pre ^ ((uint64_t)(d + 1u) << 58) ^ ((uint64_t)root * 0x9E3779B97F4A7C15ull);
    h ^= h >> 33;
    h *= 0xff51afd7ed558ccdull;
    h ^= h >> 33;
    h *= 0xc4ceb9fe1a85ec53ull;
    h ^= h >> 33;
    return h;
}
PHANT_DEV uint32_t direct_index(uint64_t kb, uint32_t root, uint32_t d, uint32_t n_roots) {
    uint32_t width = 1u, below = 0u;
    for (uint32_t t = 0; t < d; ++t) {
        below += width;
        width <<= 4;
    }
    const uint32_t pre = d ? (uint32_t)(kb >> (64u - 4u * d)) : 0u;
    return n_roots * below + root * width + pre;
}
PHANT_DEV uint32_t slot_a(uint64_t h, uint32_t mask) { return (uint32_t)h & mask; }
PHANT_DEV uint32_t slot_b(uint64_t h, uint32_t mask) { return (uint32_t)(h >> 24) & mask; }

struct Args {
    VerifyArgs v;
    uint32_t total_nodes;
    uint32_t shallow;
    uint32_t direct;
    uint32_t* dtab;
    uint64_t* table;
    uint32_t tmask;
    uint32_t* rep;
    uint2* ent;
    uint32_t stripe_cap;
    uint32_t* hdr;
    uint32_t* digest;
    uint8_t* nstat;
    uint64_t* last;
};

PHANT_DEV void beside_the_hashing() { __builtin_amdgcn_s_setprio(3); }

__global__ void __launch_bounds__(256) zero_kernel(uint4* p, size_t n16, uint32_t* fail_count, uint32_t n_roots) {
    beside_the_hashing();
    const size_t i = (size_t)blockIdx.x * 256u + threadIdx.x;
    if (i < n16) p[i] = make_uint4(0u, 0u, 0u, 0u);
    if (fail_count)
        for (size_t r = i; r < n_roots; r += (size_t)gridDim.x * 256u) fail_count[r] = 0u;
}

struct ShallowLane {
    uint32_t p, d, j, root, len;
    uint64_t kb;
    bool act;
    bool valid;
    bool group;
    bool broken;
};
PHANT_DEV ShallowLane shallow_node(const Args& a, uint32_t p, uint32_t d) {
    ShallowLane L;
    L.p = p;
    L.d = d;
    L.j = 0;
    L.root = 0;
    L.len = 0;
    L.kb = 0;
    L.act = L.valid = L.group = L.broken = false;
    if (L.p >= a.v.n) return L;
    const uint32_t first = a.v.proof_first_node[L.p], last = a.v.proof_first_node[L.p + 1];
    if (last < first) {
        L.broken = L.d == 0u;
        return L;
    }
    if (last > a.total_nodes) return L;
    const uint32_t nn = 2u * a.v.key_len, cnt = last - first;
    const uint32_t end = cnt <= nn ? cnt : nn + 1u;
    if (L.d >= end) return L;
    L.act = true;
    L.j = first + L.d;
    L.root = a.v.root_idx ? a.v.root_idx[L.p] : 0u;
    const uint64_t e = a.v.node_off[L.j + 1], b = a.v.node_off[L.j];
    if (e >= b && e <= a.v.nodes_len && e - b <= 0x7fffffffull) {
        L.valid = true;
        L.len = (uint32_t)(e - b);
    }
    L.group = L.valid && L.len >= RATE && L.root < a.v.n_roots;
    if (L.group) L.kb = key_prefix64(a.v.keys + (uint64_t)a.v.key_len * L.p, a.v.key_len);
    return L;
}
PHANT_DEV ShallowLane shallow_lane(const Args& a, uint32_t g) {
    const uint32_t p = g / a.shallow;
    return shallow_node(a, p, g - p * a.shallow);
}

PHANT_DEV void clear_launch_state(const Args& a, uint32_t g, size_t lanes) {
    const uint32_t other = HDR_STAT + HDR_STAT_WORDS * ((a.hdr[HDR_PARITY] & 1u) ^ 1u);
    for (size_t i = g; i < HDR_WORDS + HDR_STAT_WORDS; i += lanes) {
        if (i < HDR_WORDS) {
            if (i != HDR_PARITY) a.hdr[i] = 0u;
        } else {
            a.hdr[other + (i - HDR_WORDS)] = 0u;
        }
    }
    if (a.v.fail_count)
        for (size_t r = g; r < a.v.n_roots; r += lanes) a.v.fail_count[r] = 0u;
}

__global__ void __launch_bounds__(256) propose_kernel(const Args a) {
    beside_the_hashing();
    const uint32_t g = blockIdx.x * 256u + threadIdx.x;
    clear_launch_state(a, g, (size_t)gridDim.x * 256u);
    const ShallowLane L = shallow_lane(a, g);
    if (L.act) a.nstat[L.j] = 0u;
    if (!L.group) return;
    if (L.d < a.direct) {
        a.dtab[direct_index(L.kb, L.root, L.d, a.v.n_roots)] = L.j + 1u;
    } else {
        const uint64_t h = group_hash(L.kb, L.root, L.d);
        const uint64_t entry = ((uint64_t)L.p << 32) | (uint64_t)(L.j + 1u);
        a.table[slot_a(h, a.tmask)] = entry;
        a.table[slot_b(h, a.tmask)] = entry;
    }
}

PHANT_DEV bool entry_matches(const Args& a, uint64_t en, const ShallowLane& L, uint32_t& node) {
    const uint32_t pr = (uint32_t)(en >> 32), j1 = (uint32_t)en;
    if (j1 == 0u || pr >= a.v.n) return false;
    node = j1 - 1u;
    if (pr == L.p) return node == L.j;
    const uint32_t f = a.v.proof_first_node[pr], l = a.v.proof_first_node[pr + 1];
    if (l < f || l > a.total_nodes || node < f || node >= l || node - f != L.d) return false;
    if ((a.v.root_idx ? a.v.root_idx[pr] : 0u) != L.root) return false;
    return same_prefix(key_prefix64(a.v.keys + (uint64_t)a.v.key_len * pr, a.v.key_len), L.kb, L.d);
}

PHANT_DEV uint64_t ent_index(const Args& a, uint32_t cls, uint32_t stripe, uint32_t at) {
    return ((uint64_t)cls * STRIPES + stripe) * a.stripe_cap + at;
}

PHANT_DEV bool wave_bytes_equal(const uint8_t* x, const uint8_t* y, uint32_t len, uint32_t lane) {
    uint32_t diff = 0;
    const uint32_t full = len & ~15u;
    for (uint32_t o = 16u * lane; o < full; o += 1024u) {
        const uint4 p = load16u(x + o), q = load16u(y + o);
        diff |= (p.x ^ q.x) | (p.y ^ q.y) | (p.z ^ q.z) | (p.w ^ q.w);
    }
    if (lane < (len & 15u)) diff |= (uint32_t)(x[full + lane] ^ y[full + lane]);
    return __ballot(diff != 0) == 0ull;
}

constexpr int COMPARE_UNROLL = 4;

__global__ void __launch_bounds__(256) PHANT_NUM_VGPR(48) dedup_kernel(const Args a) {
    constexpr uint32_t WAVES = 4;
    __shared__ uint32_t s_cnt[WAVES][N_LIST];
    __shared__ uint32_t s_base[N_LIST];
    beside_the_hashing();
    const uint32_t tid = threadIdx.x, lane = tid & 63u, wave = tid >> 6;
    const uint32_t NT = a.total_nodes;
    if (tid < WAVES * N_LIST) (&s_cnt[0][0])[tid] = 0u;
    const ShallowLane L = shallow_lane(a, blockIdx.x * 256u + tid);
    if (L.broken) a.hdr[HDR_PFN_BROKEN] = 1u;

    const uint32_t j = L.j;
    uint32_t cand = j;
    uint64_t b = 0, cb = 0;
    if (L.group) {
        uint32_t c = j;
        if (L.d < a.direct) {
            const uint32_t t = a.dtab[direct_index(L.kb, L.root, L.d, a.v.n_roots)];
            if (t) c = t - 1u;
        } else {
            const uint64_t h = group_hash(L.kb, L.root, L.d);
            uint32_t node;
            if (entry_matches(a, a.table[slot_a(h, a.tmask)], L, node)) c = node;
            else if (entry_matches(a, a.table[slot_b(h, a.tmask)], L, node)) c = node;
        }
        if (c != j && c < NT) {
            const uint64_t c0 = a.v.node_off[c], c1 = a.v.node_off[c + 1];
            if (c1 >= c0 && c1 <= a.v.nodes_len && c1 - c0 == L.len) {
                cand = c;
                cb = c0;
                b = a.v.node_off[j];
            }
        }
    }

    const uint32_t coff = 16u * (lane & 31u);
    const bool upper = lane >= 32u;
    const uint32_t b_lo = (uint32_t)b, b_hi = (uint32_t)(b >> 32), cb_lo = (uint32_t)cb, cb_hi = (uint32_t)(cb >> 32);
    bool differs = false;
// ... 393 lines not shown
            }
            lo ^= (uint32_t)w;
            hi ^= (uint32_t)(w >> 32);
        }
        coop_permute(c, lo, hi);
        if (k + 1u == nb) {
            dlo = lo;
            dhi = hi;
        }
    }
    bool ne = false;
    if (refp && l < 4u) {
        const unsigned long long r = reinterpret_cast<const U64*>(refp + 8u * l)->v;
        ne = (uint32_t)r != dlo || (uint32_t)(r >> 32) != dhi;
    }
    const uint32_t any_bad = (uint32_t)(__ballot(bad != 0u) >> base), any_ne = (uint32_t)(__ballot(ne) >> base);
    if (active) {
        uint32_t ns = NS_HASHED | ((branch && any_bad == 0u) ? NS_CANON : 0u);
        if (refp) ns |= NS_LINK_CHECKED | (any_ne == 0u ? NS_LINK_OK : 0u);
        if (l < 4u) {
            a.digest[8ull * j + 2u * l] = dlo;
            a.digest[8ull * j + 2u * l + 1u] = dhi;
        }
        if (l == 0) {
            a.nstat[j] = (uint8_t)ns;
            const uint32_t cls = len / RATE < N_CLASS ? len / RATE : N_CLASS - 1u;
            if (stat_word != NO_STAT) atomicAdd(&a.hdr[stat_word + cls], 1u);
        }
    }
}

__global__ void __launch_bounds__(256) hash_coop_kernel(const Args a, const uint32_t levels) {
    const uint32_t tid = threadIdx.x, l = tid & 31u, base = tid & 32u;
    const uint32_t h = blockIdx.x * (blockDim.x >> 5) + (tid >> 5);
    const uint32_t p = h / levels, level = h % levels;
    uint32_t first = 0, count = 0, root = 0;
    if (p < a.v.n) {
        first = a.v.proof_first_node[p];
        const uint32_t last = a.v.proof_first_node[p + 1];
        if (last >= first && last <= a.total_nodes) count = last - first;
        if (last < first && l == 0) a.hdr[HDR_PFN_BROKEN] = 1u;
        if (a.v.root_idx) root = a.v.root_idx[p];
    }
    const uint32_t stat_word = HDR_STAT + HDR_STAT_WORDS * (a.hdr[HDR_PARITY] & 1u) + N_CLASS * (h % HDR_STAT_STRIPES);
    const CoopLane c = coop_lane(l, base, gridDim.x * (blockDim.x >> 6) <= 1024u);
    for (uint32_t d = level;; d += levels) {
        if (__ballot(d < count) == 0ull) break;
        coop_node(a, c, l, base, d < count, p, first + d, d, root, stat_word);
    }
}

PHANT_DEV void wave_node(const Args& a, const WaveLane& c, const uint32_t l, const uint32_t p, const uint32_t j, const uint32_t d, const uint32_t root,
                         const uint32_t stat_word) {
    struct __attribute__((packed, aligned(1))) U64 { unsigned long long v; };
    const uint32_t nn = 2u * a.v.key_len;
    const uint64_t e = a.v.node_off[j + 1], b = a.v.node_off[j];
    const bool active = e >= b && e <= a.v.nodes_len && e - b <= 0x7fffffffull;
    if (!active) {
        if (l == 0) a.nstat[j] = 0u;
        return;
    }
    const uint32_t len = (uint32_t)(e - b);
    const uint8_t* const ptr = a.v.nodes + b;
    const uint8_t* const key = a.v.keys + (uint64_t)a.v.key_len * p;
    const uint8_t* const refp = ref_location(a, j, d, root, (d >= 1u && d - 1u < nn) ? key_nibble(key, d - 1u) : 16u, b);
    const uint32_t nb = len / RATE + 1u;
    const bool branch = len == BRANCH_LEN;
    uint32_t lo = 0, hi = 0, bad = 0;
    for (uint32_t k = 0; k < nb; ++k) {
        if (c.word < 17u) {
            const uint32_t off = k * RATE + 8u * c.word;
            unsigned long long w = 0;
            if (off + 8u <= len) {
                w = reinterpret_cast<const U64*>(ptr + off)->v;
            } else {
#pragma unroll
                for (uint32_t t = 0; t < 8u; ++t) {
                    const uint32_t q = off + t;
                    if (q < len) w |= (unsigned long long)ptr[q] << (8u * t);
                    else if (q == len) w |= 0x01ull << (8u * t);
                }
            }
            if (k + 1u == nb && c.word == 16u) w |= 0x80ull << 56;
            if (branch) {
#pragma unroll
                for (uint32_t t = 0; t < 8u; ++t) {
                    const uint32_t q = off + t;
                    const uint32_t byte = (uint32_t)(w >> (8u * t)) & 0xffu;
                    const int want = q == 0u ? 0xf9 : q == 1u ? 0x02 : q == 2u ? 0x11 : q == BRANCH_LEN - 1u ? 0x80 : (q < BRANCH_LEN && (q - 3u) % 33u == 0u) ? 0xa0 : -1;
                    if (want >= 0 && byte != (uint32_t)want) bad = 1u;
                }
            }
            lo ^= (uint32_t)w;
            hi ^= (uint32_t)(w >> 32);
        }
        wave_permute(c, lo, hi);
    }
    bool ne = false;
    if (refp && l < 4u) {
        const unsigned long long r = reinterpret_cast<const U64*>(refp + 8u * l)->v;
        ne = (uint32_t)r != lo || (uint32_t)(r >> 32) != hi;
    }
    const bool any_bad = __ballot(bad != 0u) != 0ull, any_ne = __ballot(ne) != 0ull;
    uint32_t ns = NS_HASHED | ((branch && !any_bad) ? NS_CANON : 0u);
    if (refp) ns |= NS_LINK_CHECKED | (!any_ne ? NS_LINK_OK : 0u);
    if (l < 4u) {
        a.digest[8ull * j + 2u * l] = lo;
        a.digest[8ull * j + 2u * l + 1u] = hi;
    }
    if (l == 0) {
        a.nstat[j] = (uint8_t)ns;
        const uint32_t cls = len / RATE < N_CLASS ? len / RATE : N_CLASS - 1u;
        if (stat_word != NO_STAT) atomicAdd(&a.hdr[stat_word + cls], 1u);
    }
}

__global__ void __launch_bounds__(256) hash_wave_kernel(const Args a, const uint32_t levels) {
    const uint32_t tid = threadIdx.x, l = tid & 63u;
    const uint32_t h = blockIdx.x * (blockDim.x >> 6) + (tid >> 6);
    const uint32_t p = h / levels, level = h % levels;
    if (p >= a.v.n) return;
    const uint32_t first = a.v.proof_first_node[p], last = a.v.proof_first_node[p + 1];
    uint32_t count = 0;
    if (last >= first && last <= a.total_nodes) count = last - first;
    if (last < first && l == 0) a.hdr[HDR_PFN_BROKEN] = 1u;
    const uint32_t root = a.v.root_idx ? a.v.root_idx[p] : 0u;
    const uint32_t stat_word = HDR_STAT + HDR_STAT_WORDS * (a.hdr[HDR_PARITY] & 1u) + N_CLASS * (h % HDR_STAT_STRIPES);
    const WaveLane c = wave_lane(l);
    for (uint32_t d = level; d < count; d += levels) wave_node(a, c, l, p, first + d, d, root, stat_word);
}

__global__ void __launch_bounds__(256, 4) hash_list_kernel(const Args a) {
    __builtin_amdgcn_s_setprio(2);
    const uint32_t waves = gridDim.x * 4u;
    uint32_t q = (uint32_t)__builtin_amdgcn_readfirstlane(blockIdx.x * 4u + (threadIdx.x >> 6));
    for (;;) {
        uint32_t lane = threadIdx.x & 63u;
        PHANT_PIN_VGPR(lane);
        const uint32_t chunks = list_role(a, q, lane);
        q += waves;
        if (q >= chunks) break;
        __builtin_amdgcn_s_setprio(2);
    }
}

enum : uint32_t { LINK_GENERIC = 0, LINK_FAST = 1, LINK_HASH_OK = 2, LINK_BAD_HASH = 3 };

PHANT_DEV uint32_t code_of(uint32_t ns, bool has_nibble) {
    if (!(ns & NS_HASHED) || !(ns & NS_LINK_CHECKED)) return LINK_GENERIC;
    if (!(ns & NS_LINK_OK)) return LINK_BAD_HASH;
    return (has_nibble && (ns & NS_CANON)) ? LINK_FAST : LINK_HASH_OK;
}


template <bool DIRECT>
__global__ void __launch_bounds__(256) walk_kernel(const Args a) {
    __shared__ uint32_t s_stage[256 * WALK_SLOT_DW];
    beside_the_hashing();
    const uint32_t i = blockIdx.x * 256u + threadIdx.x;
    const bool in = i < a.v.n;
    uint32_t status = PHANT_PROOF_PRESENT;
    uint32_t r = 0;
    if (in) {
        uint32_t* const slot = s_stage + threadIdx.x * WALK_SLOT_DW;
        const uint8_t* const slot_node = reinterpret_cast<const uint8_t*>(slot);
        const uint8_t* const nodes_end = a.v.nodes + a.v.nodes_len;
        uint64_t voff = 0;
        uint32_t vlen = 0;
        const uint32_t first = a.v.proof_first_node[i], last = a.v.proof_first_node[i + 1];
        const uint64_t rec = i < a.total_nodes ? a.last[i] : 0ull;
        r = a.v.root_idx ? a.v.root_idx[i] : 0u;
        if (last < first || last > a.total_nodes || r >= a.v.n_roots) {
            status = PHANT_PROOF_BAD_INPUT;
        } else if (last == first) {
            uint32_t rw[8];
            GlobalBytes rb{a.v.roots + 32ull * r};
#pragma unroll
            for (int k = 0; k < 8; ++k) rw[k] = rb.u32(4 * k);
            status = is_empty_root(rw) ? PHANT_PROOF_ABSENT : PHANT_PROOF_INVALID_EMPTY;
        } else if (a.hdr[HDR_PFN_BROKEN] != 0u) {
            status = STATUS_NEEDS_SLOW;
        } else {
            const uint8_t* const key = a.v.keys + (uint64_t)a.v.key_len * i;
            const uint32_t nn = 2u * a.v.key_len;
            uint32_t sx = 0;
            if constexpr (!DIRECT) {
                const uint32_t cnt = last - first, end = cnt <= nn ? cnt : nn + 1u;
                sx = end < a.shallow ? end : a.shallow;
            }
            const uint8_t* const slot_key = reinterpret_cast<const uint8_t*>(slot + WALK_STAGE_BYTES / 4);
            const bool key_in_lds = a.v.key_len <= WALK_KEY_BYTES;
            WalkState w;
            w.pos = 0;
            w.status = PHANT_PROOF_BAD_INPUT;
            w.value_pay = w.value_len = w.ref_pay = w.ref_total = 0;
            uint32_t used = first;
            status = 0xffffffffu;

            bool hash_known = false;
            bool recorded = false;
            uint32_t rprev = 0;
            for (bool run = true; run && used < last;) {
                const uint32_t base = used, dbase = used - first;
                const uint8_t* lp = a.nstat + base;
                const uint32_t c0 = load4u(lp), c1 = load4u(lp + 4);
                uint32_t rj[8], nsr[8], rpar[8];
                if constexpr (!DIRECT) {
                    if (dbase < sx) {
                        const uint8_t* rp = reinterpret_cast<const uint8_t*>(a.rep + base);
                        const uint4 r0 = load16u(rp), r1 = load16u(rp + 16);
                        rj[0] = r0.x; rj[1] = r0.y; rj[2] = r0.z; rj[3] = r0.w;
                        rj[4] = r1.x; rj[5] = r1.y; rj[6] = r1.z; rj[7] = r1.w;
#pragma unroll
                        for (int u = 0; u < 8; ++u) {
                            const bool sh = dbase + u < sx && base + u < last && rj[u] < a.total_nodes;
                            rj[u] = sh ? rj[u] : base + u;
                        }
#pragma unroll
                        for (int u = 0; u < 8; ++u) {
                            const bool copy = rj[u] != base + u;
                            nsr[u] = copy ? a.nstat[rj[u]] : 0u;
                            rpar[u] = (copy && rj[u] >= 1u && dbase + u >= 1u) ? a.rep[rj[u] - 1u] : 0xffffffffu;
                        }
                    } else {
#pragma unroll
                        for (int u = 0; u < 8; ++u) {
                            rj[u] = base + u;
                            nsr[u] = 0u;
                            rpar[u] = 0xffffffffu;
                        }
                    }
                }
#pragma unroll
                for (int u = 0; u < 8; ++u) {
                    if (!run || used >= last) continue;
                    const uint32_t own = ((u < 4 ? c0 : c1) >> (8 * (u & 3))) & 0xffu;
                    uint32_t c, me = used;
                    if constexpr (DIRECT) {
                        c = code_of(own, w.pos < nn);
                    } else {
                        me = rj[u];
                        if (me == used) c = code_of(own, w.pos < nn);
                        else if (used == first || rpar[u] == rprev) c = code_of(nsr[u], w.pos < nn);
                        else if (!(nsr[u] & NS_HASHED)) c = LINK_GENERIC;
                        else {
                            const uint8_t* rb = a.v.nodes + a.v.node_off[used - 1u] + (4u + 33u * key_nibble(key, w.pos - 1u));
                            const uint4 w0 = load16u(rb), w1 = load16u(rb + 16);
                            const uint4* dg = reinterpret_cast<const uint4*>(a.digest + 8ull * me);
                            const uint4 d0 = dg[0], d1 = dg[1];
                            const uint32_t diff = (d0.x ^ w0.x) | (d0.y ^ w0.y) | (d0.z ^ w0.z) | (d0.w ^ w0.w) |
                                                  (d1.x ^ w1.x) | (d1.y ^ w1.y) | (d1.z ^ w1.z) | (d1.w ^ w1.w);
                            c = diff ? LINK_BAD_HASH : ((w.pos < nn && (nsr[u] & NS_CANON)) ? LINK_FAST : LINK_HASH_OK);
                        }
                    }
                    if (c == LINK_FAST) {
                        ++used;
                        w.pos += 1;
                        rprev = me;
                    } else {
                        run = false;
                        if (c == LINK_BAD_HASH) status = PHANT_PROOF_BAD_HASH;
                        else hash_known = c == LINK_HASH_OK;
                        recorded = me == used && (own & NS_LAST) != 0u;
                    }
                }
            }

            if (status == 0xffffffffu && hash_known && recorded && used + 1u == last && last_pos(rec) == w.pos &&
                last_code(rec) != LAST_NONE) {
                ++used;
                if (last_code(rec) == LAST_PRESENT) {
                    status = PHANT_PROOF_PRESENT;
                    voff = last_value_off(rec);
                    vlen = last_value_len(rec);
                } else {
                    status = PHANT_PROOF_ABSENT;
                }
            }
            if (status == 0xffffffffu && key_in_lds) {
                uint8_t* kdst = reinterpret_cast<uint8_t*>(slot + WALK_STAGE_BYTES / 4);
                for (uint32_t t = 0; t < a.v.key_len; ++t) kdst[t] = key[t];
            }

            uint32_t want[8] = {0, 0, 0, 0, 0, 0, 0, 0};
            if (status == 0xffffffffu && !hash_known) {
                if (used == first) {
                    GlobalBytes rb{a.v.roots + 32ull * r};
#pragma unroll
                    for (int k = 0; k < 8; ++k) want[k] = rb.u32(4 * k);
                } else {
                    const uint32_t nibp = key_nibble(key, w.pos - 1u);
                    const uint8_t* rb = a.v.nodes + a.v.node_off[used - 1u] + (4u + 33u * nibp);
                    const uint4 r0 = load16u(rb), r1 = load16u(rb + 16);
                    want[0] = r0.x; want[1] = r0.y; want[2] = r0.z; want[3] = r0.w;
                    want[4] = r1.x; want[5] = r1.y; want[6] = r1.z; want[7] = r1.w;
                }
            }
            bool by_hash = true;
            const uint8_t* cur = nullptr;
            uint32_t cur_len = 0, opened = 0;
            const uint8_t* staged_from = nullptr;
            for (;;) {
                if (status != 0xffffffffu) break;
                ++opened;
                if (by_hash) {
                    if (used == last) {
                        status = PHANT_PROOF_MISSING_NODE;
                        break;
                    }
                    const uint32_t j = used;
                    const uint64_t b = a.v.node_off[j], e = a.v.node_off[j + 1];
                    if (e < b || e > a.v.nodes_len || e - b > 0x7fffffffull) {
                        status = PHANT_PROOF_BAD_INPUT;
                        break;
                    }
                    cur = a.v.nodes + b;
                    cur_len = (uint32_t)(e - b);
                    ++used;
                    if (hash_known) {
                        hash_known = false;
                    } else {
                        uint32_t rj = j;
                        if constexpr (!DIRECT) {
                            if (j - first < sx) rj = a.rep[j];
                        }
                        if (!(rj < a.total_nodes && (a.nstat[rj] & NS_HASHED))) {
                            status = STATUS_NEEDS_SLOW;
                            break;
                        }
                        const uint4* dg = reinterpret_cast<const uint4*>(a.digest + 8ull * rj);
                        const uint4 d0 = dg[0], d1 = dg[1];
                        const uint32_t diff = (d0.x ^ want[0]) | (d0.y ^ want[1]) | (d0.z ^ want[2]) | (d0.w ^ want[3]) |
                                              (d1.x ^ want[4]) | (d1.y ^ want[5]) | (d1.z ^ want[6]) | (d1.w ^ want[7]);
                        if (diff) {
                            status = PHANT_PROOF_BAD_HASH;
                            break;
                        }
                        if ((a.nstat[rj] & NS_CANON) && w.pos < nn) {
                            const uint8_t* rb = cur + (4u + 33u * key_nibble(key, w.pos));
                            const uint4 r0 = load16u(rb), r1 = load16u(rb + 16);
                            want[0] = r0.x; want[1] = r0.y; want[2] = r0.z; want[3] = r0.w;
                            want[4] = r1.x; want[5] = r1.y; want[6] = r1.z; want[7] = r1.w;
                            w.pos += 1;
                            continue;
                        }
                    }
                    staged_from = nullptr;
                    const uint32_t padded = (cur_len + 15u) & ~15u;
                    if (cur_len <= WALK_STAGE_BYTES && cur + padded <= nodes_end) {
                        for (uint32_t o = 0; o < padded; o += 16u) {
                            const uint4 q = load16u(cur + o);
                            slot[o / 4u] = q.x;
                            slot[o / 4u + 1u] = q.y;
                            slot[o / 4u + 2u] = q.z;
                            slot[o / 4u + 3u] = q.w;
                        }
                        staged_from = cur;
                    }
                }
                auto step_from = [&](const uint8_t* nb, const uint8_t* kp) __attribute__((always_inline)) -> uint32_t {
                    GlobalBytes nd{nb};
                    const uint32_t st = walk_node(nd, cur_len, kp, nn, w);
                    if (st == STEP_HASH) {
#pragma unroll
                        for (int k = 0; k < 8; ++k) want[k] = nd.u32(w.ref_pay + 4 * k);
                    }
                    return st;
                };
                uint32_t step;
                if (!key_in_lds) step = step_from(cur, key);
                else if (staged_from) step = step_from(slot_node + (cur - staged_from), slot_key);
                else step = step_from(cur, slot_key);
                if (step == STEP_DONE) break;
                if (step == STEP_HASH) {
                    by_hash = true;
                } else {
                    cur = cur + w.ref_pay;
                    cur_len = w.ref_total;
                    by_hash = false;
                }
            }
            if (opened > 1u) atomicAdd(&a.hdr[HDR_OPENED], opened);
            if (status == 0xffffffffu) {
                status = w.status;
                if (status == PHANT_PROOF_PRESENT || status == PHANT_PROOF_ABSENT) {
                    if (used != last) {
                        status = PHANT_PROOF_EXTRA_NODES;
                    } else if (status == PHANT_PROOF_PRESENT) {
                        voff = (uint64_t)(cur - a.v.nodes) + w.value_pay;
                        vlen = w.value_len;
                    }
                }
            }
        }
        if (status == STATUS_NEEDS_SLOW) {
            atomicAdd(&a.hdr[HDR_SLOW], 1u);
            status = verify_one(a.v, i, voff, vlen);
        }
        a.v.status[i] = (uint8_t)status;
        if (a.v.value_off) a.v.value_off[i] = voff;
        if (a.v.value_len) a.v.value_len[i] = vlen;
    }
    if (blockIdx.x == 0 && threadIdx.x == 0) a.hdr[HDR_PARITY] ^= 1u;
    if (a.v.fail_count) {
        const bool bad = in && !(status == PHANT_PROOF_PRESENT || status == PHANT_PROOF_ABSENT);
        if (a.v.root_idx == nullptr || a.v.n_roots == 1) {
            const unsigned long long m = __ballot(bad);
            if ((threadIdx.x & 63u) == 0 && m) atomicAdd(&a.v.fail_count[0], (uint32_t)__popcll(m));
        } else if (bad) {
            atomicAdd(&a.v.fail_count[r < a.v.n_roots ? r : 0u], 1u);
        }
    }
}

__global__ void __launch_bounds__(256) stream_read_kernel(const uint4* __restrict__ p, size_t n16, uint32_t* sink, size_t mask) {
    const size_t stride = (size_t)gridDim.x * 256u;
    size_t i = (size_t)blockIdx.x * 256u + threadIdx.x;
    uint4 acc = make_uint4(0u, 0u, 0u, 0u);
    for (; i + 7u * stride < n16; i += 8u * stride) {
        uint4 v[8];
#pragma unroll
        for (int u = 0; u < 8; ++u) v[u] = p[(i + (size_t)u * stride) & mask];
#pragma unroll
        for (int u = 0; u < 8; ++u) {
            acc.x ^= v[u].x;
            acc.y ^= v[u].y;
            acc.z ^= v[u].z;
            acc.w ^= v[u].w;
        }
    }
    for (; i < n16; i += stride) {
        const uint4 v = p[i & mask];
        acc.x ^= v.x;
        acc.y ^= v.y;
        acc.z ^= v.z;
        acc.w ^= v.w;
    }
    const uint32_t x = acc.x ^ acc.y ^ acc.z ^ acc.w;
    if (x == 0x9e3779b9u && sink) sink[blockIdx.x & 255u] = x;
}

static size_t rnd256(size_t x) { return (x + 255) / 256 * 256; }

constexpr uint64_t HASH_EVERYTHING_BELOW_BYTES = 72000000ull;

static uint32_t shallow_levels(uint32_t n, uint32_t n_roots, uint64_t nodes_len, int32_t forced) {
    if (forced >= 0) return (uint32_t)forced < MAX_SHALLOW ? (uint32_t)forced : MAX_SHALLOW;
    if (n < 2 || nodes_len < HASH_EVERYTHING_BELOW_BYTES) return 0;
    uint64_t n_eff = n;
    if (n_roots > 1u) {
        uint64_t r = 1;
        while ((r + 1) * (r + 1) <= n_roots) ++r;
        n_eff = n / r ? n / r : 1;
    }
    uint32_t s = 1;
    uint64_t groups = 16;
    while (s < MAX_SHALLOW && groups <= 4ull * n_eff) {
        ++s;
        groups *= 16;
    }
    return s;
}

constexpr uint64_t DIRECT_MAX_ENTRIES = 1ull << 21;
static uint32_t direct_levels(uint32_t n_roots, uint32_t shallow, uint64_t& entries) {
    uint32_t d = 0;
    uint64_t below = 0, width = 1;
    entries = 0;
    while (d < shallow && (below + width) * n_roots <= DIRECT_MAX_ENTRIES) {
        below += width;
        width *= 16;
        ++d;
        entries = below * n_roots;
    }
    return d;
}

static uint32_t table_entries(uint32_t n, uint32_t n_roots, uint32_t direct, uint32_t shallow, uint32_t total_nodes) {
    uint64_t per_root = 0, g = 1;
    for (uint32_t d = 0; d < shallow && per_root < (1ull << 40); ++d, g *= 16)
        if (d >= direct) per_root += g;
    uint64_t groups = per_root * (n_roots ? n_roots : 1u);
    const uint64_t by_nodes = (uint64_t)n * (shallow - direct) < total_nodes ? (uint64_t)n * (shallow - direct) : total_nodes;
    if (groups > by_nodes) groups = by_nodes;
    uint32_t t = 1024;
    while (t < 4 * groups && t < (1u << 26)) t <<= 1;
    return t;
}

struct Layout {
    size_t nstat, dtab, table, rep, ent, digest, last, end;
    uint32_t stripe_cap;
};
static Layout layout(uint32_t total_nodes, uint32_t te, uint64_t direct_entries, uint64_t lanes) {
    const size_t tn = total_nodes;
    Layout l;
    const uint64_t wgs = (lanes + 255u) / 256u;
    l.stripe_cap = (uint32_t)((wgs + STRIPES - 1u) / STRIPES * 256u);
    size_t p = HEADER_BYTES;
    l.nstat = p;  p += rnd256(tn + 16);
    l.dtab = p;   p += rnd256((size_t)direct_entries * 4);
    l.table = p;  p += rnd256((size_t)te * 8);
    l.rep = p;    p += rnd256(tn * 4 + 64);
    l.ent = p;    p += rnd256((size_t)N_LIST * STRIPES * l.stripe_cap * 8u);
    l.digest = p; p += rnd256(tn * 32);
    l.last = p;   p += rnd256(tn * 8);
    l.end = p + 1024;
    return l;
}

size_t workspace_bytes(uint32_t total_nodes) {
    uint32_t t = 1024;
    while (t < 4ull * total_nodes && t < (1u << 26)) t <<= 1;
    const uint64_t lanes = (uint64_t)total_nodes + 256u * STRIPES;
    return layout(total_nodes, t, DIRECT_MAX_ENTRIES, lanes).end;
}

static void bind(Args& a, uint8_t* ws, const Layout& l, uint32_t te) {
    a.hdr = reinterpret_cast<uint32_t*>(ws);
    a.nstat = ws + l.nstat;
    a.dtab = reinterpret_cast<uint32_t*>(ws + l.dtab);
    a.table = reinterpret_cast<uint64_t*>(ws + l.table);
    a.tmask = te - 1u;
    a.rep = reinterpret_cast<uint32_t*>(ws + l.rep);
    a.ent = reinterpret_cast<uint2*>(ws + l.ent);
    a.stripe_cap = l.stripe_cap;
    a.digest = reinterpret_cast<uint32_t*>(ws + l.digest);
    a.last = reinterpret_cast<uint64_t*>(ws + l.last);
}

}

size_t verify_workspace_bytes(uint32_t total_nodes) { return v3::workspace_bytes(total_nodes); }

hipError_t launch_mpt_verify(const VerifyArgs& v_in, uint32_t total_nodes, uint8_t* ws, int32_t dedup_levels,
                                hipStream_t st, const FlatSide* side, const VerifyTune& tune) {
    using namespace v3;
    VerifyArgs v = v_in;
    v.total_nodes = total_nodes;
    if (v.n == 0) return hipSuccess;
    Args a;
    a.v = v;
    a.total_nodes = total_nodes;
    a.shallow = shallow_levels(v.n, v.n_roots, v.nodes_len, dedup_levels);
    while (a.shallow && (uint64_t)v.n * a.shallow > (uint64_t)total_nodes + 256u * STRIPES) --a.shallow;
    if (tune.last_shallow) *tune.last_shallow = total_nodes ? a.shallow : 0u;
    uint64_t direct_entries = 0;
    a.direct = direct_levels(v.n_roots, a.shallow, direct_entries);
    const uint32_t te = table_entries(v.n, v.n_roots, a.direct, a.shallow, total_nodes);
    const uint64_t lanes = (uint64_t)v.n * a.shallow;
    const Layout l = layout(total_nodes, te, direct_entries, lanes);
    bind(a, ws, l, te);
    hipError_t e = hipSuccess;
    const uint32_t pg = (v.n + 255u) / 256u;
    const uint32_t wpl = (v.n + 63u) / 64u;
    const uint64_t avg_len = total_nodes ? (total_nodes + v.n - 1u) / v.n : 0u;
    const bool uniform = avg_len != 0u && 8ull * total_nodes + v.n >= 8ull * avg_len * v.n;
    const uint64_t depths = avg_len + (uniform ? 0u : 1u);
    const uint32_t deep_levels = depths <= a.shallow ? 1u : (uint32_t)(depths - a.shallow < DEEP_LEVELS ? depths - a.shallow : DEEP_LEVELS);
    const bool ride = uniform && avg_len >= a.shallow + 2ull && avg_len - a.shallow <= DEEP_LEVELS;
    const uint32_t deep_rows = ride ? deep_levels - 1u : deep_levels;
    const uint32_t ride_d = ride ? a.shallow + deep_rows - 1u : NO_RIDE;
    const uint32_t deep_wgs = (wpl * deep_rows + 3u) / 4u;
    if (tune.last_form) *tune.last_form = (a.shallow == 0u || total_nodes == 0u) ? 0u : 1u;
    if (a.shallow == 0u || total_nodes == 0u) {
        a.shallow = 0;
        const size_t zero_n16 = l.dtab / 16;
        hipLaunchKernelGGL(zero_kernel, dim3((uint32_t)((zero_n16 + 255) / 256)), dim3(256), 0, st, reinterpret_cast<uint4*>(ws),
                           zero_n16, v.fail_count, v.n_roots);
        const uint64_t halves = (uint64_t)v.n * deep_levels;
        if (total_nodes && total_nodes <= tune.coop_max && !tune.no_coop && halves <= 4ull * COOP_MAX_NODES)
            if (halves <= WAVE_MAX_NODES && !tune.no_wave) {
                if (halves <= 512u) hipLaunchKernelGGL(hash_wave_kernel, dim3((uint32_t)halves), dim3(64), 0, st, a, deep_levels);
                else hipLaunchKernelGGL(hash_wave_kernel, dim3((uint32_t)((halves + 3u) / 4u)), dim3(256), 0, st, a, deep_levels);
            } else if (halves <= 1024u) {
                hipLaunchKernelGGL(hash_coop_kernel, dim3((uint32_t)((halves + 1u) / 2u)), dim3(64), 0, st, a, deep_levels);
            } else {
                hipLaunchKernelGGL(hash_coop_kernel, dim3((uint32_t)((halves + 7u) / 8u)), dim3(256), 0, st, a, deep_levels);
            }
        else if (total_nodes)
            hipLaunchKernelGGL(hash_deep_kernel<true>, dim3(deep_wgs), dim3(256), 0, st, a, wpl, deep_rows, ride_d);
        hipLaunchKernelGGL(walk_kernel<true>, dim3(pg), dim3(256), 0, st, a);
        return hipGetLastError();
    }
    const uint32_t sg = (uint32_t)((lanes + 255u) / 256u);
    const bool two = side && side->stream && side->fork && side->join && !tune.serial;
    hipStream_t hs = two ? side->stream : st;
    uint64_t listed = 0, groups = (uint64_t)(v.n_roots ? v.n_roots : 1u);
    for (uint32_t d = 0; d < a.shallow; ++d) {
        listed += groups < v.n ? groups : v.n;
        if (groups < v.n) groups *= 16u;
    }
    listed += listed / 8u;
    if (listed > lanes) listed = lanes;
    if (listed > total_nodes) listed = total_nodes;
    uint32_t list_wgs = (uint32_t)((listed + 255u) / 256u) + (N_QUEUE + 3u) / 4u;
    if (tune.list_wgs_cap && list_wgs > tune.list_wgs_cap) list_wgs = tune.list_wgs_cap;
    const uint32_t hash_lds = two ? tune.hash_lds : 0u;
    if (two) {
        if ((e = hipEventRecord(side->fork, st)) != hipSuccess) return e;
        if ((e = hipStreamWaitEvent(side->stream, side->fork, 0)) != hipSuccess) return e;
    }
    hipEvent_t* const kev = (!two && tune.serial) ? tune.kernel_ev : nullptr;
    auto mark = [&](int i) {
        if (kev && e == hipSuccess) e = hipEventRecord(kev[i], st);
    };
    if (tune.diag) {
        const bool three = two && side->stream2 && side->join2;
        hipStream_t h2 = three ? side->stream2 : st;
        if (two) {
            if ((e = hipEventRecord(side->fork, st)) != hipSuccess) return e;
            if ((e = hipStreamWaitEvent(side->stream, side->fork, 0)) != hipSuccess) return e;
            if (three && (e = hipStreamWaitEvent(side->stream2, side->fork, 0)) != hipSuccess) return e;
        }
        if (tune.diag & 1u) {
            const uint32_t lds = tune.diag == 3u ? hash_lds : 0u;
            hipLaunchKernelGGL(hash_deep_kernel<false>, dim3(deep_wgs), dim3(256), lds, hs, a, wpl, deep_rows, ride_d);
            hipLaunchKernelGGL(hash_list_kernel, dim3(list_wgs), dim3(256), lds ? lds + 8192u : 0u, st, a);
        }
        if (tune.diag & 2u) {
            const uint32_t wgs = tune.diag_stream_wgs ? tune.diag_stream_wgs : 2048u;
            size_t mask = ~(size_t)0;
            if (tune.diag_stream_mb) {
                size_t r16 = (size_t)tune.diag_stream_mb << 16;
                while (r16 > v.nodes_len / 16u) r16 >>= 1;
                mask = r16 ? r16 - 1u : 0u;
            }
            hipLaunchKernelGGL(stream_read_kernel, dim3(wgs), dim3(256), 0, h2, reinterpret_cast<const uint4*>(v.nodes),
                               (size_t)(v.nodes_len / 16u), tune.diag_sink, mask);
        }
        if (two) {
            if ((e = hipEventRecord(side->join, side->stream)) != hipSuccess) return e;
            if ((e = hipStreamWaitEvent(st, side->join, 0)) != hipSuccess) return e;
            if (three) {
                if ((e = hipEventRecord(side->join2, side->stream2)) != hipSuccess) return e;
                if ((e = hipStreamWaitEvent(st, side->join2, 0)) != hipSuccess) return e;
            }
        }
        return hipGetLastError();
    }
    mark(0);
    hipLaunchKernelGGL(propose_kernel, dim3(sg), dim3(256), 0, st, a);
    mark(1);
    hipLaunchKernelGGL(hash_deep_kernel<false>, dim3(deep_wgs), dim3(256), hash_lds, hs, a, wpl, deep_rows, ride_d);
    mark(2);
    if (two && (e = hipEventRecord(side->join, side->stream)) != hipSuccess) return e;
    hipLaunchKernelGGL(dedup_kernel, dim3(sg), dim3(256), 0, st, a);
    mark(3);
    hipLaunchKernelGGL(hash_list_kernel, dim3(list_wgs), dim3(256), hash_lds ? hash_lds + 8192u : 0u, st, a);
    mark(4);
    if (two && (e = hipStreamWaitEvent(st, side->join, 0)) != hipSuccess) return e;
    hipLaunchKernelGGL(walk_kernel<false>, dim3(pg), dim3(256), 0, st, a);
    mark(5);
    if (e != hipSuccess) return e;
    return hipGetLastError();
}

void verify_stats_from_header(const uint32_t* hdr, uint32_t hashed[8]) {
    using namespace v3;
    uint32_t lists[N_LIST];
    for (uint32_t c = 0; c < N_LIST; ++c) {
        lists[c] = 0;
        for (uint32_t s = 0; s < STRIPES; ++s) lists[c] += hdr[HDR_CUR + 32u * s + c];
    }
    const uint32_t buf = (hdr[HDR_PARITY] & 1u) ^ 1u;
    for (uint32_t c = 0; c < N_CLASS; ++c) {
        hashed[c] = lists[c];
        for (uint32_t s = 0; s < HDR_STAT_STRIPES; ++s) hashed[c] += hdr[HDR_STAT + HDR_STAT_WORDS * buf + N_CLASS * s + c];
    }
    hashed[BRANCH_LEN / RATE] += lists[LIST_B532];
}
void verify_tier_stats_from_header(const uint32_t* hdr, uint32_t out[4]) {
    using namespace v3;
    out[0] = out[1] = out[2] = out[3] = 0;
    for (uint32_t c = 0; c < N_LIST; ++c) {
        uint32_t cnt = 0;
        for (uint32_t s = 0; s < STRIPES; ++s) cnt += hdr[HDR_CUR + 32u * s + c];
        out[0] += cnt;
        out[1] += cnt * (c == LIST_B532 ? BRANCH_LEN / RATE + 1u : c + 1u);
    }
    const uint32_t buf = (hdr[HDR_PARITY] & 1u) ^ 1u;
    for (uint32_t c = 0; c < N_CLASS; ++c)
        for (uint32_t s = 0; s < HDR_STAT_STRIPES; ++s) {
            const uint32_t cnt = hdr[HDR_STAT + HDR_STAT_WORDS * buf + N_CLASS * s + c];
            out[2] += cnt;
            out[3] += cnt * (c + 1u);
        }
}
void verify_paths_from_header(const uint32_t* hdr, uint32_t out[2]) {
    out[0] = hdr[v3::HDR_SLOW];
    out[1] = hdr[v3::HDR_OPENED];
}

}
```

Baseline: 576.3 million proofs/s.

## Split walk into lean settle kernel plus compacted rest kernel for hard proofs

The single walk kernel is split into a low-register settle_kernel that resolves the common fast-path proofs without LDS staging, and a rest_kernel that processes only proofs handed on through striped pending lists in the header. The aim is to raise occupancy for the fast path and avoid carrying the large LDS slot and slow-path register footprint for every proof. The cost is an extra launch, atomics for compaction, a pending buffer in the workspace, and a fallback full scan if the buffer overflows. A diagnostic knob caps rest grid size and a query reports how many proofs were handed on.

```diff
diff --git a/include/phant_gpu_diag.h b/include/phant_gpu_diag.h
--- a/include/phant_gpu_diag.h
+++ b/include/phant_gpu_diag.h
@@ -13,6 +13,7 @@
 PHANT_API int32_t phant_verify_stats(phant_ctx *ctx, uint32_t hashed[8]);
 PHANT_API int32_t phant_verify_path_stats(phant_ctx *ctx, uint32_t out[2]);
 PHANT_API int32_t phant_verify_tier_stats(phant_ctx *ctx, uint32_t out[5]);
+PHANT_API int32_t phant_verify_handed_on(phant_ctx *ctx, uint32_t *proofs);
 PHANT_API int32_t phant_verify_form(phant_ctx *ctx, uint32_t *form);
 #define PHANT_VERIFY_KERNEL_STAGES 5
 PHANT_API int32_t phant_verify_kernel_ms(phant_ctx *ctx, float ms[PHANT_VERIFY_KERNEL_STAGES]);
@@ -69,7 +70,8 @@
     PHANT_DIAG_ADVANCE_ESTIMATE_BYTES,
     PHANT_DIAG_VERIFY_LIST_WGS,
     PHANT_DIAG_RANGES_NO_LEAF_PASS,
-    PHANT_DIAG_RANGES_ITEMS_PER_RANGE
+    PHANT_DIAG_RANGES_ITEMS_PER_RANGE,
+    PHANT_DIAG_VERIFY_REST_WGS
 };
 PHANT_API int32_t phant_diag_set(phant_ctx *ctx, uint32_t knob, int64_t value);
 
diff --git a/phant_amd/_lib.py b/phant_amd/_lib.py
--- a/phant_amd/_lib.py
+++ b/phant_amd/_lib.py
@@ -139,6 +139,7 @@
     "phant_diag_set": (_i32, [_vp, _u32, C.c_int64]),
     "phant_verify_kernel_ms": (_i32, [_vp, C.POINTER(C.c_float * 5)]),
     "phant_verify_form": (_i32, [_vp, C.POINTER(C.c_uint32)]),
+    "phant_verify_handed_on": (_i32, [_vp, C.POINTER(C.c_uint32)]),
     "phant_verify_bound_experiment": (_i32, [_vp, _vp, _u32, _vp, _vp, _u32, _vp, _u64, _vp, _u32, _vp, _u32, _vp, _u32,
                                             C.POINTER(C.c_float * 3)]),
     "phant_verify_stats": (_i32, [_vp, C.POINTER(C.c_uint32 * 8)]),
diff --git a/phant_amd/context.py b/phant_amd/context.py
--- a/phant_amd/context.py
+++ b/phant_amd/context.py
@@ -73,7 +73,8 @@
         "trie_no_side", "trie_side_min_keys", "trie_ahead_max_keys", "trie_side_lds", "trie_fallback_grid", "trie_slot_blocks",
         "trie_no_coop", "trie_coop_max", "trie_no_wave", "trie_join_in_stream", "sort_no_fallback", "sort_prefix_bits",
         "sort_repair_bits", "nodeset_wave_max", "trie_small_max_keys", "code_hash_form", "poststate_raw_slot_keys",
-        "advance_estimate_bytes", "verify_list_wgs", "ranges_no_leaf_pass", "ranges_items_per_range"))}
+        "advance_estimate_bytes", "verify_list_wgs", "ranges_no_leaf_pass", "ranges_items_per_range",
+        "verify_rest_wgs"))}
 
     def diag_set(self, knob: str, value: int):
         self.check(self._lib.phant_diag_set(self._h, self.DIAG[knob], int(value)))
@@ -131,6 +132,11 @@
         self.check(self._lib.phant_verify_path_stats(self._h, C.byref(out)))
         return int(out[0]), int(out[1])
 
+    def verify_handed_on(self) -> int:
+        out = C.c_uint32(0)
+        self.check(self._lib.phant_verify_handed_on(self._h, C.byref(out)))
+        return int(out.value)
+
     def close(self):
         if getattr(self, "_h", None):
             if not getattr(self, "_borrowed", False):
diff --git a/phant_amd/csrc/capi.hip b/phant_amd/csrc/capi.hip
--- a/phant_amd/csrc/capi.hip
+++ b/phant_amd/csrc/capi.hip
@@ -344,6 +344,19 @@
     uint32_t hdr[phant::VERIFY_HEADER_WORDS];
     HIP_TRY(c, hipMemcpy(hdr, c->dv.base, sizeof(hdr), hipMemcpyDeviceToHost));
     phant::verify_paths_from_header(hdr, out);
+    return PHANT_OK;
+}
+
+int32_t phant_verify_handed_on(phant_ctx* c, uint32_t* proofs) {
+    if (!c || !proofs) return PHANT_E_INVALID_ARG;
+    *proofs = 0;
+    if (!c->dv.base) return PHANT_OK;
+    DeviceGuard g(c->device);
+    HIP_TRY(c, hipStreamSynchronize(c->stream));
+    if (c->side.stream) HIP_TRY(c, hipStreamSynchronize(c->side.stream));
+    uint32_t hdr[phant::VERIFY_HEADER_WORDS];
+    HIP_TRY(c, hipMemcpy(hdr, c->dv.base, sizeof(hdr), hipMemcpyDeviceToHost));
+    *proofs = phant::verify_handed_on_from_header(hdr);
     return PHANT_OK;
 }
 
@@ -447,6 +460,7 @@
         case PHANT_DIAG_POSTSTATE_RAW_SLOT_KEYS: c->post_raw_slot_keys = value != 0; return PHANT_OK;
         case PHANT_DIAG_ADVANCE_ESTIMATE_BYTES: c->advance_estimate = value > 0 ? (uint64_t)value : 0u; return PHANT_OK;
         case PHANT_DIAG_VERIFY_LIST_WGS: c->tune.list_wgs_cap = (uint32_t)(value < 0 ? 0 : value > (1 << 20) ? (1 << 20) : value); return PHANT_OK;
+        case PHANT_DIAG_VERIFY_REST_WGS: c->tune.rest_wgs_cap = (uint32_t)(value < 0 ? 0 : value > (1 << 20) ? (1 << 20) : value); return PHANT_OK;
         case PHANT_DIAG_RANGES_NO_LEAF_PASS: c->ranges_no_leaf_pass = value != 0; return PHANT_OK;
         case PHANT_DIAG_RANGES_ITEMS_PER_RANGE: c->ranges_items_per_range = value < 0 ? -1 : value > 1922 ? 1922 : value; return PHANT_OK;
         default: return fail(c, PHANT_E_INVALID_ARG, "diag_set: no such knob");
diff --git a/phant_amd/csrc/capi_guard_capi.inc b/phant_amd/csrc/capi_guard_capi.inc
--- a/phant_amd/csrc/capi_guard_capi.inc
+++ b/phant_amd/csrc/capi_guard_capi.inc
@@ -506,6 +506,12 @@
     catch (...) { return phant_impl::guard_failed(ctx, PHANT_E_DEVICE); }
 }
 
+int32_t phant_verify_handed_on(phant_ctx *ctx, uint32_t *proofs) {
+    try { return phant_impl::phant_verify_handed_on(ctx, proofs); }
+    catch (const std::bad_alloc&) { return phant_impl::guard_failed(ctx, PHANT_E_OOM); }
+    catch (...) { return phant_impl::guard_failed(ctx, PHANT_E_DEVICE); }
+}
+
 int32_t phant_verify_form(phant_ctx *ctx, uint32_t *form) {
     try { return phant_impl::phant_verify_form(ctx, form); }
     catch (const std::bad_alloc&) { return phant_impl::guard_failed(ctx, PHANT_E_OOM); }
diff --git a/phant_amd/csrc/launch.h b/phant_amd/csrc/launch.h
--- a/phant_amd/csrc/launch.h
+++ b/phant_amd/csrc/launch.h
@@ -62,6 +62,7 @@
     bool no_wave = false;
     uint32_t* last_form = nullptr;
     uint32_t list_wgs_cap = 0;
+    uint32_t rest_wgs_cap = 0;
     uint32_t diag = 0;
     uint32_t* diag_sink = nullptr;
     uint32_t diag_stream_wgs = 0;
@@ -74,6 +75,7 @@
 void verify_stats_from_header(const uint32_t* hdr, uint32_t hashed[8]);
 void verify_tier_stats_from_header(const uint32_t* hdr, uint32_t out[4]);
 void verify_paths_from_header(const uint32_t* hdr, uint32_t out[2]);
+uint32_t verify_handed_on_from_header(const uint32_t* hdr);
 struct NodesetTune {
     uint32_t form = 1;
     uint32_t order = 0;
diff --git a/phant_amd/csrc/mpt_verify_v3.hip b/phant_amd/csrc/mpt_verify_v3.hip
--- a/phant_amd/csrc/mpt_verify_v3.hip
+++ b/phant_amd/csrc/mpt_verify_v3.hip
@@ -12,13 +12,17 @@
 constexpr uint32_t HDR_PFN_BROKEN = 9;
 constexpr uint32_t HDR_SLOW = 10;
 constexpr uint32_t HDR_OPENED = 11;
+constexpr uint32_t HDR_PEND_OVERFLOW = 12;
 constexpr uint32_t HDR_PARITY = 15;
 constexpr uint32_t HDR_STAT = 1024;
 constexpr uint32_t HDR_STAT_STRIPES = 16;
 constexpr uint32_t HDR_STAT_WORDS = HDR_STAT_STRIPES * N_CLASS;
 constexpr uint32_t HDR_STAT_END = HDR_STAT + 2u * HDR_STAT_WORDS;
 constexpr uint32_t HDR_CUR = 256;
+constexpr uint32_t HDR_PEND = 512;
+constexpr uint32_t PEND_STRIPES = 8;
 constexpr uint32_t HDR_WORDS = 768;
+static_assert(HDR_CUR + 32u * STRIPES <= HDR_PEND && HDR_PEND + 32u * PEND_STRIPES <= HDR_WORDS, "cursor lines apart, and cleared per launch");
 constexpr size_t HEADER_BYTES = 8192;
 static_assert(HDR_STAT_END <= VERIFY_HEADER_WORDS && 4u * VERIFY_HEADER_WORDS <= HEADER_BYTES,
               "capi.hip copies VERIFY_HEADER_WORDS words back for the statistics");
@@ -76,6 +80,8 @@
     uint32_t* digest;
     uint8_t* nstat;
     uint64_t* last;
+    uint32_t* pend;
+    uint32_t pend_cap;
 };
 
 PHANT_DEV void beside_the_hashing() { __builtin_amdgcn_s_setprio(3); }
@@ -775,138 +781,244 @@
     return (has_nibble && (ns & NS_CANON)) ? LINK_FAST : LINK_HASH_OK;
 }
 
-
+PHANT_DEV uint32_t shallow_end(const Args& a, uint32_t first, uint32_t last) {
+    const uint32_t nn = 2u * a.v.key_len, cnt = last - first, end = cnt <= nn ? cnt : nn + 1u;
+    return end < a.shallow ? end : a.shallow;
+}
+
+PHANT_DEV uint64_t decode_leaf_here(const Args& a, const uint32_t j, const uint8_t* __restrict__ key, const uint32_t pos) {
+    const uint64_t b = a.v.node_off[j], e = a.v.node_off[j + 1];
+    if (e < b || e > a.v.nodes_len || e - b >= RATE) return 0ull;
+    const uint8_t* const p = a.v.nodes + b;
+    uint32_t d[RATE_DWORDS];
+#pragma unroll
+    for (uint32_t k = 0; k < RATE_DWORDS; ++k) d[k] = 0u;
+    if (b + 48u <= a.v.nodes_len) {
+        const uint4 q0 = load16u(p), q1 = load16u(p + 16), q2 = load16u(p + 32);
+        d[0] = q0.x; d[1] = q0.y; d[2] = q0.z; d[3] = q0.w;
+        d[4] = q1.x; d[5] = q1.y; d[6] = q1.z; d[7] = q1.w;
+        d[8] = q2.x; d[9] = q2.y; d[10] = q2.z; d[11] = q2.w;
+    } else {
+#pragma unroll
+        for (uint32_t k = 0; k < 12u; ++k) {
+#pragma unroll
+            for (uint32_t q = 0; q < 4u; ++q)
+                if (b + 4u * k + q < a.v.nodes_len) d[k] |= (uint32_t)p[4u * k + q] << (8u * q);
+        }
+    }
+    return decode_last_leaf(d, (uint32_t)(e - b), key, a.v.key_len, pos, b);
+}
+
+constexpr uint32_t UNSETTLED = 0xffffffffu;
+struct Settled {
+    uint32_t status;
+    uint32_t root, first, last;
+    uint32_t used;
+    uint32_t pos;
+    bool hash_known;
+    uint64_t voff;
+    uint32_t vlen;
+};
 template <bool DIRECT>
-__global__ void __launch_bounds__(256) walk_kernel(const Args a) {
-    __shared__ uint32_t s_stage[256 * WALK_SLOT_DW];
+PHANT_DEV Settled settle_proof(const Args& a, const uint32_t i) {
+    Settled s;
+    s.status = UNSETTLED;
+    s.used = s.pos = s.vlen = 0;
+    s.voff = 0;
+    s.hash_known = false;
+    const uint32_t first = a.v.proof_first_node[i], last = a.v.proof_first_node[i + 1];
+    s.first = first;
+    s.last = last;
+    const uint64_t rec = i < a.total_nodes ? a.last[i] : 0ull;
+    const uint32_t r = a.v.root_idx ? a.v.root_idx[i] : 0u;
+    s.root = r;
+    if (last < first || last > a.total_nodes || r >= a.v.n_roots) {
+        s.status = PHANT_PROOF_BAD_INPUT;
+        return s;
+    }
+    if (last == first) {
+        uint32_t rw[8];
+        GlobalBytes rb{a.v.roots + 32ull * r};
+#pragma unroll
+        for (int k = 0; k < 8; ++k) rw[k] = rb.u32(4 * k);
+        s.status = is_empty_root(rw) ? PHANT_PROOF_ABSENT : PHANT_PROOF_INVALID_EMPTY;
+        return s;
+    }
+    if (a.hdr[HDR_PFN_BROKEN] != 0u) {
+        s.status = STATUS_NEEDS_SLOW;
+        return s;
+    }
+    const uint8_t* const key = a.v.keys + (uint64_t)a.v.key_len * i;
+    const uint32_t nn = 2u * a.v.key_len;
+    uint32_t sx = 0;
+    if constexpr (!DIRECT) sx = shallow_end(a, first, last);
+    uint32_t used = first, pos = 0, status = UNSETTLED;
+
+    bool hash_known = false;
+    bool recorded = false;
+    uint32_t rprev = 0;
+    for (bool run = true; run && used < last;) {
+        const uint32_t base = used, dbase = used - first;
+        const uint8_t* lp = a.nstat + base;
+        const uint32_t c0 = load4u(lp), c1 = load4u(lp + 4);
+        uint32_t rj[8], nsr[8], rpar[8];
+        if constexpr (!DIRECT) {
+            if (dbase < sx) {
+                const uint8_t* rp = reinterpret_cast<const uint8_t*>(a.rep + base);
+                const uint4 r0 = load16u(rp), r1 = load16u(rp + 16);
+                rj[0] = r0.x; rj[1] = r0.y; rj[2] = r0.z; rj[3] = r0.w;
+                rj[4] = r1.x; rj[5] = r1.y; rj[6] = r1.z; rj[7] = r1.w;
+#pragma unroll
+                for (int u = 0; u < 8; ++u) {
+                    const bool sh = dbase + u < sx && base + u < last && rj[u] < a.total_nodes;
+                    rj[u] = sh ? rj[u] : base + u;
+                }
+#pragma unroll
+                for (int u = 0; u < 8; ++u) {
+                    const bool copy = rj[u] != base + u;
+                    nsr[u] = copy ? a.nstat[rj[u]] : 0u;
+                    rpar[u] = (copy && rj[u] >= 1u && dbase + u >= 1u) ? a.rep[rj[u] - 1u] : 0xffffffffu;
+                }
+            } else {
+#pragma unroll
+                for (int u = 0; u < 8; ++u) {
+                    rj[u] = base + u;
+                    nsr[u] = 0u;
+                    rpar[u] = 0xffffffffu;
+                }
+            }
+        }
+#pragma unroll
+        for (int u = 0; u < 8; ++u) {
+            if (!run || used >= last) continue;
+            const uint32_t own = ((u < 4 ? c0 : c1) >> (8 * (u & 3))) & 0xffu;
+            uint32_t c, me = used;
+            if constexpr (DIRECT) {
+                c = code_of(own, pos < nn);
+            } else {
+                me = rj[u];
+                if (me == used) c = code_of(own, pos < nn);
+                else if (used == first || rpar[u] == rprev) c = code_of(nsr[u], pos < nn);
+                else if (!(nsr[u] & NS_HASHED)) c = LINK_GENERIC;
+                else {
+                    const uint8_t* rb = a.v.nodes + a.v.node_off[used - 1u] + (4u + 33u * key_nibble(key, pos - 1u));
+                    const uint4 w0 = load16u(rb), w1 = load16u(rb + 16);
+                    const uint4* dg = reinterpret_cast<const uint4*>(a.digest + 8ull * me);
+                    const uint4 d0 = dg[0], d1 = dg[1];
+                    const uint32_t diff = (d0.x ^ w0.x) | (d0.y ^ w0.y) | (d0.z ^ w0.z) | (d0.w ^ w0.w) |
+                                          (d1.x ^ w1.x) | (d1.y ^ w1.y) | (d1.z ^ w1.z) | (d1.w ^ w1.w);
+                    c = diff ? LINK_BAD_HASH : ((pos < nn && (nsr[u] & NS_CANON)) ? LINK_FAST : LINK_HASH_OK);
+                }
+            }
+            if (c == LINK_FAST) {
+                ++used;
+                pos += 1;
+                rprev = me;
+            } else {
+                run = false;
+                if (c == LINK_BAD_HASH) status = PHANT_PROOF_BAD_HASH;
+                else hash_known = c == LINK_HASH_OK;
+                recorded = me == used && (own & NS_LAST) != 0u;
+            }
+        }
+    }
+
+    if (status == UNSETTLED && hash_known && used + 1u == last) {
+        const uint64_t word = recorded ? rec : decode_leaf_here(a, used, key, pos);
+        if (last_pos(word) == pos && last_code(word) != LAST_NONE) {
+            ++used;
+            if (last_code(word) == LAST_PRESENT) {
+                status = PHANT_PROOF_PRESENT;
+                s.voff = last_value_off(word);
+                s.vlen = last_value_len(word);
+            } else {
+                status = PHANT_PROOF_ABSENT;
+            }
+        }
+    }
+    s.status = status;
+    s.used = used;
+    s.pos = pos;
+    s.hash_known = hash_known;
+    return s;
+}
+
+PHANT_DEV void count_verdict(const Args& a, const bool counted, const uint32_t status, const uint32_t r) {
+    if (!a.v.fail_count) return;
+    const bool bad = counted && !(status == PHANT_PROOF_PRESENT || status == PHANT_PROOF_ABSENT);
+    if (a.v.root_idx == nullptr || a.v.n_roots == 1) {
+        const unsigned long long m = __ballot(bad);
+        if ((threadIdx.x & 63u) == 0 && m) atomicAdd(&a.v.fail_count[0], (uint32_t)__popcll(m));
+    } else if (bad) {
+        atomicAdd(&a.v.fail_count[r < a.v.n_roots ? r : 0u], 1u);
+    }
+}
+
+PHANT_DEV uint32_t pend_cursor(uint32_t stripe) { return HDR_PEND + 32u * stripe; }
+
+template <bool DIRECT>
+__global__ void __launch_bounds__(256) PHANT_NUM_VGPR(64) settle_kernel(const Args a) {
     beside_the_hashing();
-    const uint32_t i = blockIdx.x * 256u + threadIdx.x;
+    const uint32_t i = blockIdx.x * 256u + threadIdx.x, lane = threadIdx.x & 63u;
     const bool in = i < a.v.n;
-    uint32_t status = PHANT_PROOF_PRESENT;
-    uint32_t r = 0;
+    uint32_t status = PHANT_PROOF_PRESENT, r = 0;
+    bool hand = false;
     if (in) {
-        uint32_t* const slot = s_stage + threadIdx.x * WALK_SLOT_DW;
-        const uint8_t* const slot_node = reinterpret_cast<const uint8_t*>(slot);
-        const uint8_t* const nodes_end = a.v.nodes + a.v.nodes_len;
-        uint64_t voff = 0;
-        uint32_t vlen = 0;
-        const uint32_t first = a.v.proof_first_node[i], last = a.v.proof_first_node[i + 1];
-        const uint64_t rec = i < a.total_nodes ? a.last[i] : 0ull;
-        r = a.v.root_idx ? a.v.root_idx[i] : 0u;
-        if (last < first || last > a.total_nodes || r >= a.v.n_roots) {
-            status = PHANT_PROOF_BAD_INPUT;
-        } else if (last == first) {
-            uint32_t rw[8];
-            GlobalBytes rb{a.v.roots + 32ull * r};
-#pragma unroll
-            for (int k = 0; k < 8; ++k) rw[k] = rb.u32(4 * k);
-            status = is_empty_root(rw) ? PHANT_PROOF_ABSENT : PHANT_PROOF_INVALID_EMPTY;
-        } else if (a.hdr[HDR_PFN_BROKEN] != 0u) {
-            status = STATUS_NEEDS_SLOW;
-        } else {
+        const Settled s = settle_proof<DIRECT>(a, i);
+        status = s.status;
+        r = s.root;
+        hand = status == UNSETTLED || status == STATUS_NEEDS_SLOW;
+        if (!hand) {
+            a.v.status[i] = (uint8_t)status;
+            if (a.v.value_off) a.v.value_off[i] = s.voff;
+            if (a.v.value_len) a.v.value_len[i] = s.vlen;
+        }
+    }
+    const unsigned long long m = __ballot(hand);
+    const uint32_t stripe = (i >> 6) % PEND_STRIPES;
+    uint32_t at = 0;
+    if (lane == 0 && m) at = atomicAdd(&a.hdr[pend_cursor(stripe)], (uint32_t)__popcll(m));
+    at = lane_u32(at, 0u) + (uint32_t)__popcll(m & ((1ull << lane) - 1ull));
+    if (hand) {
+        a.v.status[i] = (uint8_t)STATUS_NEEDS_SLOW;
+        if (at < a.pend_cap) a.pend[(size_t)stripe * a.pend_cap + at] = i;
+        else a.hdr[HDR_PEND_OVERFLOW] = 1u;
+    }
+    count_verdict(a, in && !hand, status, r);
+}
+
+template <bool DIRECT>
+PHANT_DEV void rest_proof(const Args& a, const bool have, const uint32_t i, uint32_t* const slot) {
+    uint32_t status = PHANT_PROOF_PRESENT, r = 0;
+    if (have) {
+        const Settled s = settle_proof<DIRECT>(a, i);
+        status = s.status;
+        r = s.root;
+        uint64_t voff = s.voff;
+        uint32_t vlen = s.vlen;
+        if (status == UNSETTLED) {
+            const uint32_t first = s.first, last = s.last;
+            const uint8_t* const slot_node = reinterpret_cast<const uint8_t*>(slot);
+            const uint8_t* const nodes_end = a.v.nodes + a.v.nodes_len;
             const uint8_t* const key = a.v.keys + (uint64_t)a.v.key_len * i;
             const uint32_t nn = 2u * a.v.key_len;
             uint32_t sx = 0;
-            if constexpr (!DIRECT) {
-                const uint32_t cnt = last - first, end = cnt <= nn ? cnt : nn + 1u;
-                sx = end < a.shallow ? end : a.shallow;
-            }
+            if constexpr (!DIRECT) sx = shallow_end(a, first, last);
             const uint8_t* const slot_key = reinterpret_cast<const uint8_t*>(slot + WALK_STAGE_BYTES / 4);
             const bool key_in_lds = a.v.key_len <= WALK_KEY_BYTES;
             WalkState w;
-            w.pos = 0;
+            w.pos = s.pos;
             w.status = PHANT_PROOF_BAD_INPUT;
             w.value_pay = w.value_len = w.ref_pay = w.ref_total = 0;
-            uint32_t used = first;
-            status = 0xffffffffu;
-
-            bool hash_known = false;
-            bool recorded = false;
-            uint32_t rprev = 0;
-            for (bool run = true; run && used < last;) {
-                const uint32_t base = used, dbase = used - first;
-                const uint8_t* lp = a.nstat + base;
-                const uint32_t c0 = load4u(lp), c1 = load4u(lp + 4);
-                uint32_t rj[8], nsr[8], rpar[8];
-                if constexpr (!DIRECT) {
-                    if (dbase < sx) {
-                        const uint8_t* rp = reinterpret_cast<const uint8_t*>(a.rep + base);
-                        const uint4 r0 = load16u(rp), r1 = load16u(rp + 16);
-                        rj[0] = r0.x; rj[1] = r0.y; rj[2] = r0.z; rj[3] = r0.w;
-                        rj[4] = r1.x; rj[5] = r1.y; rj[6] = r1.z; rj[7] = r1.w;
-#pragma unroll
-                        for (int u = 0; u < 8; ++u) {
-                            const bool sh = dbase + u < sx && base + u < last && rj[u] < a.total_nodes;
-                            rj[u] = sh ? rj[u] : base + u;
-                        }
-#pragma unroll
-                        for (int u = 0; u < 8; ++u) {
-                            const bool copy = rj[u] != base + u;
-                            nsr[u] = copy ? a.nstat[rj[u]] : 0u;
-                            rpar[u] = (copy && rj[u] >= 1u && dbase + u >= 1u) ? a.rep[rj[u] - 1u] : 0xffffffffu;
-                        }
-                    } else {
-#pragma unroll
-                        for (int u = 0; u < 8; ++u) {
-                            rj[u] = base + u;
-                            nsr[u] = 0u;
-                            rpar[u] = 0xffffffffu;
-                        }
-                    }
-                }
-#pragma unroll
-                for (int u = 0; u < 8; ++u) {
-                    if (!run || used >= last) continue;
-                    const uint32_t own = ((u < 4 ? c0 : c1) >> (8 * (u & 3))) & 0xffu;
-                    uint32_t c, me = used;
-                    if constexpr (DIRECT) {
-                        c = code_of(own, w.pos < nn);
-                    } else {
-                        me = rj[u];
-                        if (me == used) c = code_of(own, w.pos < nn);
-                        else if (used == first || rpar[u] == rprev) c = code_of(nsr[u], w.pos < nn);
-                        else if (!(nsr[u] & NS_HASHED)) c = LINK_GENERIC;
-                        else {
-                            const uint8_t* rb = a.v.nodes + a.v.node_off[used - 1u] + (4u + 33u * key_nibble(key, w.pos - 1u));
-                            const uint4 w0 = load16u(rb), w1 = load16u(rb + 16);
-                            const uint4* dg = reinterpret_cast<const uint4*>(a.digest + 8ull * me);
-                            const uint4 d0 = dg[0], d1 = dg[1];
-                            const uint32_t diff = (d0.x ^ w0.x) | (d0.y ^ w0.y) | (d0.z ^ w0.z) | (d0.w ^ w0.w) |
-                                                  (d1.x ^ w1.x) | (d1.y ^ w1.y) | (d1.z ^ w1.z) | (d1.w ^ w1.w);
-                            c = diff ? LINK_BAD_HASH : ((w.pos < nn && (nsr[u] & NS_CANON)) ? LINK_FAST : LINK_HASH_OK);
-                        }
-                    }
-                    if (c == LINK_FAST) {
-                        ++used;
-                        w.pos += 1;
-                        rprev = me;
-                    } else {
-                        run = false;
-                        if (c == LINK_BAD_HASH) status = PHANT_PROOF_BAD_HASH;
-                        else hash_known = c == LINK_HASH_OK;
-                        recorded = me == used && (own & NS_LAST) != 0u;
-                    }
-                }
-            }
-
-            if (status == 0xffffffffu && hash_known && recorded && used + 1u == last && last_pos(rec) == w.pos &&
-                last_code(rec) != LAST_NONE) {
-                ++used;
-                if (last_code(rec) == LAST_PRESENT) {
-                    status = PHANT_PROOF_PRESENT;
-                    voff = last_value_off(rec);
-                    vlen = last_value_len(rec);
-                } else {
-                    status = PHANT_PROOF_ABSENT;
-                }
-            }
-            if (status == 0xffffffffu && key_in_lds) {
+            uint32_t used = s.used;
+            bool hash_known = s.hash_known;
+            if (key_in_lds) {
                 uint8_t* kdst = reinterpret_cast<uint8_t*>(slot + WALK_STAGE_BYTES / 4);
                 for (uint32_t t = 0; t < a.v.key_len; ++t) kdst[t] = key[t];
             }
 
             uint32_t want[8] = {0, 0, 0, 0, 0, 0, 0, 0};
-            if (status == 0xffffffffu && !hash_known) {
+            if (!hash_known) {
                 if (used == first) {
                     GlobalBytes rb{a.v.roots + 32ull * r};
 #pragma unroll
@@ -924,7 +1036,6 @@
             uint32_t cur_len = 0, opened = 0;
             const uint8_t* staged_from = nullptr;
             for (;;) {
-                if (status != 0xffffffffu) break;
                 ++opened;
                 if (by_hash) {
                     if (used == last) {
@@ -1004,7 +1115,7 @@
                 }
             }
             if (opened > 1u) atomicAdd(&a.hdr[HDR_OPENED], opened);
-            if (status == 0xffffffffu) {
+            if (status == UNSETTLED) {
                 status = w.status;
                 if (status == PHANT_PROOF_PRESENT || status == PHANT_PROOF_ABSENT) {
                     if (used != last) {
@@ -1024,17 +1135,39 @@
         if (a.v.value_off) a.v.value_off[i] = voff;
         if (a.v.value_len) a.v.value_len[i] = vlen;
     }
-    if (blockIdx.x == 0 && threadIdx.x == 0) a.hdr[HDR_PARITY] ^= 1u;
-    if (a.v.fail_count) {
-        const bool bad = in && !(status == PHANT_PROOF_PRESENT || status == PHANT_PROOF_ABSENT);
-        if (a.v.root_idx == nullptr || a.v.n_roots == 1) {
-            const unsigned long long m = __ballot(bad);
-            if ((threadIdx.x & 63u) == 0 && m) atomicAdd(&a.v.fail_count[0], (uint32_t)__popcll(m));
-        } else if (bad) {
-            atomicAdd(&a.v.fail_count[r < a.v.n_roots ? r : 0u], 1u);
-        }
-    }
-}
+    count_verdict(a, have, status, r);
+}
+
+template <bool DIRECT>
+__global__ void __launch_bounds__(64) rest_kernel(const Args a) {
+    __shared__ uint32_t s_stage[64 * WALK_SLOT_DW];
+    beside_the_hashing();
+    const uint32_t lane = threadIdx.x, waves = gridDim.x;
+    uint32_t* const slot = s_stage + lane * WALK_SLOT_DW;
+    const uint32_t cnt = lane < PEND_STRIPES ? a.hdr[pend_cursor(lane)] : 0u;
+    if (__ballot(a.hdr[HDR_PEND_OVERFLOW] != 0u) == 0ull) {
+        uint32_t longest = 0;
+        for (uint32_t s = 0; s < PEND_STRIPES; ++s) {
+            const uint32_t c = lane_u32(cnt, s);
+            longest = c > longest ? c : longest;
+        }
+        const uint64_t chunks = (uint64_t)PEND_STRIPES * ((longest + 63u) / 64u);
+        for (uint64_t q = blockIdx.x; q < chunks; q += waves) {
+            const uint32_t s = (uint32_t)(q % PEND_STRIPES), at = (uint32_t)(q / PEND_STRIPES) * 64u + lane;
+            const bool have = at < lane_u32(cnt, s) && at < a.pend_cap;
+            const uint32_t i = have ? a.pend[(size_t)s * a.pend_cap + at] : 0u;
+            rest_proof<DIRECT>(a, have, i, slot);
+        }
+    } else {
+        for (uint64_t base = 64ull * blockIdx.x; base < a.v.n; base += 64ull * waves) {
+            const uint32_t i = (uint32_t)(base + lane);
+            const bool have = base + lane < a.v.n && a.v.status[i] == (uint8_t)STATUS_NEEDS_SLOW;
+            rest_proof<DIRECT>(a, have, i, slot);
+        }
+    }
+    if (blockIdx.x == 0 && lane == 0) a.hdr[HDR_PARITY] ^= 1u;
+}
+
 
 __global__ void __launch_bounds__(256) stream_read_kernel(const uint4* __restrict__ p, size_t n16, uint32_t* sink, size_t mask) {
     const size_t stride = (size_t)gridDim.x * 256u;
@@ -1066,6 +1199,7 @@
 static size_t rnd256(size_t x) { return (x + 255) / 256 * 256; }
 
 constexpr uint64_t HASH_EVERYTHING_BELOW_BYTES = 72000000ull;
+constexpr uint32_t REST_WGS_RIDE = 8;
 
 static uint32_t shallow_levels(uint32_t n, uint32_t n_roots, uint64_t nodes_len, int32_t forced) {
     if (forced >= 0) return (uint32_t)forced < MAX_SHALLOW ? (uint32_t)forced : MAX_SHALLOW;
@@ -1112,8 +1246,8 @@
 }
 
 struct Layout {
-    size_t nstat, dtab, table, rep, ent, digest, last, end;
-    uint32_t stripe_cap;
+    size_t nstat, dtab, table, rep, ent, digest, last, pend, end;
+    uint32_t stripe_cap, pend_cap;
 };
 static Layout layout(uint32_t total_nodes, uint32_t te, uint64_t direct_entries, uint64_t lanes) {
     const size_t tn = total_nodes;
@@ -1128,6 +1262,8 @@
     l.ent = p;    p += rnd256((size_t)N_LIST * STRIPES * l.stripe_cap * 8u);
     l.digest = p; p += rnd256(tn * 32);
     l.last = p;   p += rnd256(tn * 8);
+    l.pend_cap = (uint32_t)((tn + 64u * PEND_STRIPES - 1u) / (64u * PEND_STRIPES) * 64u);
+    l.pend = p;   p += rnd256((size_t)PEND_STRIPES * l.pend_cap * 4u);
     l.end = p + 1024;
     return l;
 }
@@ -1150,6 +1286,8 @@
     a.stripe_cap = l.stripe_cap;
     a.digest = reinterpret_cast<uint32_t*>(ws + l.digest);
     a.last = reinterpret_cast<uint64_t*>(ws + l.last);
+    a.pend = reinterpret_cast<uint32_t*>(ws + l.pend);
+    a.pend_cap = l.pend_cap;
 }
 
 }
@@ -1185,6 +1323,12 @@
     const uint32_t deep_rows = ride ? deep_levels - 1u : deep_levels;
     const uint32_t ride_d = ride ? a.shallow + deep_rows - 1u : NO_RIDE;
     const uint32_t deep_wgs = (wpl * deep_rows + 3u) / 4u;
+    auto rest_grid = [&](bool rides) {
+        const uint64_t per_proof = ((uint64_t)v.n + 63u) / 64u;
+        uint32_t g = (uint32_t)(rides && per_proof > REST_WGS_RIDE ? REST_WGS_RIDE : per_proof);
+        if (tune.rest_wgs_cap && g > tune.rest_wgs_cap) g = tune.rest_wgs_cap;
+        return g;
+    };
     if (tune.last_form) *tune.last_form = (a.shallow == 0u || total_nodes == 0u) ? 0u : 1u;
     if (a.shallow == 0u || total_nodes == 0u) {
         a.shallow = 0;
@@ -1192,7 +1336,8 @@
         hipLaunchKernelGGL(zero_kernel, dim3((uint32_t)((zero_n16 + 255) / 256)), dim3(256), 0, st, reinterpret_cast<uint4*>(ws),
                            zero_n16, v.fail_count, v.n_roots);
         const uint64_t halves = (uint64_t)v.n * deep_levels;
-        if (total_nodes && total_nodes <= tune.coop_max && !tune.no_coop && halves <= 4ull * COOP_MAX_NODES)
+        const bool coop = total_nodes && total_nodes <= tune.coop_max && !tune.no_coop && halves <= 4ull * COOP_MAX_NODES;
+        if (coop)
             if (halves <= WAVE_MAX_NODES && !tune.no_wave) {
                 if (halves <= 512u) hipLaunchKernelGGL(hash_wave_kernel, dim3((uint32_t)halves), dim3(64), 0, st, a, deep_levels);
                 else hipLaunchKernelGGL(hash_wave_kernel, dim3((uint32_t)((halves + 3u) / 4u)), dim3(256), 0, st, a, deep_levels);
@@ -1203,7 +1348,8 @@
             }
         else if (total_nodes)
             hipLaunchKernelGGL(hash_deep_kernel<true>, dim3(deep_wgs), dim3(256), 0, st, a, wpl, deep_rows, ride_d);
-        hipLaunchKernelGGL(walk_kernel<true>, dim3(pg), dim3(256), 0, st, a);
+        hipLaunchKernelGGL(settle_kernel<true>, dim3(pg), dim3(256), 0, st, a);
+        hipLaunchKernelGGL(rest_kernel<true>, dim3(rest_grid(ride && !coop)), dim3(64), 0, st, a);
         return hipGetLastError();
     }
     const uint32_t sg = (uint32_t)((lanes + 255u) / 256u);
@@ -1273,7 +1419,8 @@
     hipLaunchKernelGGL(hash_list_kernel, dim3(list_wgs), dim3(256), hash_lds ? hash_lds + 8192u : 0u, st, a);
     mark(4);
     if (two && (e = hipStreamWaitEvent(st, side->join, 0)) != hipSuccess) return e;
-    hipLaunchKernelGGL(walk_kernel<false>, dim3(pg), dim3(256), 0, st, a);
+    hipLaunchKernelGGL(settle_kernel<false>, dim3(pg), dim3(256), 0, st, a);
+    hipLaunchKernelGGL(rest_kernel<false>, dim3(rest_grid(ride)), dim3(64), 0, st, a);
     mark(5);
     if (e != hipSuccess) return e;
     return hipGetLastError();
@@ -1314,5 +1461,10 @@
     out[0] = hdr[v3::HDR_SLOW];
     out[1] = hdr[v3::HDR_OPENED];
 }
-
-}
+uint32_t verify_handed_on_from_header(const uint32_t* hdr) {
+    uint32_t handed = 0;
+    for (uint32_t s = 0; s < v3::PEND_STRIPES; ++s) handed += hdr[v3::HDR_PEND + 32u * s];
+    return handed;
+}
+
+}
```

Measured after the change: 571.5 million proofs/s. About the same (-0.8%).
